# Coder-Yu/SELFRec

Hardware: NVIDIA H100
Metric: XSimGCL yelp2018 train steps/sec (higher is better)
Workload: dtype f32

## Files before the change

selfrec_b200/csrc/common.cuh:

```cuda
#pragma once
#include <cuda_runtime.h>
#include <stdint.h>
#include <stdio.h>
#include <atomic>
#include <functional>
#include <utility>
#include "selfrec_b200.h"

#define SRB_FULL_MASK 0xffffffffu

namespace srb {

void set_error(const char* fmt, ...);
extern std::atomic<long long> g_launches;

inline int check_cuda(cudaError_t e, const char* what) {
  if (e != cudaSuccess) {
    set_error("%s: %s", what, cudaGetErrorString(e));
    return SRB_ERR_CUDA;
  }
  return SRB_OK;
}

inline int post_launch(const char* what) {
  g_launches.fetch_add(1, std::memory_order_relaxed);
  return check_cuda(cudaPeekAtLastError(), what);
}

__device__ __forceinline__ void pdl_wait() { asm volatile("griddepcontrol.wait;" ::: "memory"); }
__device__ __forceinline__ void pdl_trigger() { asm volatile("griddepcontrol.launch_dependents;" ::: "memory"); }

bool pdl_active();

template <typename... KArgs, typename... Args>
inline int launch_kernel(void (*kernel)(KArgs...), dim3 grid, dim3 block, size_t smem, cudaStream_t st, const char* what,
                         Args&&... args) {
  cudaLaunchAttribute attr[1];
  attr[0].id = cudaLaunchAttributeProgrammaticStreamSerialization;
  attr[0].val.programmaticStreamSerializationAllowed = 1;
  cudaLaunchConfig_t cfg = {};
  cfg.gridDim = grid;
  cfg.blockDim = block;
  cfg.dynamicSmemBytes = smem;
  cfg.stream = st;
  cfg.attrs = attr;
  cfg.numAttrs = pdl_active() ? 1 : 0;
  const cudaError_t e = cudaLaunchKernelEx(&cfg, kernel, std::forward<Args>(args)...);
  g_launches.fetch_add(1, std::memory_order_relaxed);
  return check_cuda(e, what);
}

#define SRB_REQUIRE(cond, ...)            \
  do {                                    \
    if (!(cond)) {                        \
      srb::set_error(__VA_ARGS__);        \
      return SRB_ERR_ARG;                 \
    }                                     \
  } while (0)

#define SRB_TRY(expr)                     \
  do {                                    \
    int _rc = (expr);                     \
    if (_rc != SRB_OK) return _rc;        \
  } while (0)

int sm_count();
long long l2_bytes();

struct ScatterSeg {
  const float* src;
  const int32_t* rows;
  const int32_t* n_dev;
  int32_t n;
  int32_t row_off;
  float scale;
  int32_t mod, rem;
  int32_t item_min;
  int32_t item_off;
};
struct ScatterSegs {
  int count;
  ScatterSeg s[16];
};
int scatter_segments(float* dst, int d, const ScatterSegs& segs, cudaStream_t st);

struct SeedRows {
  int32_t user_off[3], item_off[3];
  int32_t user_mod, user_rem;
  int32_t item_min;
};
struct SeedGrads {
  const int32_t* batch;
  int cap, d;
  const float *emb, *l2;
  const float *nce_u[2], *nce_i[2];
  const int32_t *cat, *n_cat;
};
int seed_segments(int model, int n_layers, int layer_cl, const SeedGrads& g, const SeedRows& r, ScatterSegs& segs);
int step_begin(int32_t* step, float* scalars, double lr, double b1, double b2, int32_t* words, int n_words, const int32_t* batch, int cap,
               int d, float* seed, int n_seed, const SeedRows& r, cudaStream_t st);

struct LossRows {
  const int32_t* batch;
  const int32_t *u, *i, *j;
  int32_t item_off;
  const int32_t *uq_u, *uq_i;
  int32_t uq_off[2];
  const int32_t *cat, *n_cat;
  const int32_t* cat_id;
};
struct LossBufs {
  float *g_emb, *g_l2;
  float* g_nce;
  size_t nce_plane;
  float *bpr_scratch, *bpr_losses, *nce_losses;
  void* nce_ws;
  int64_t nce_ws_bytes;
  float* losses;
};
struct ForkRes;
int step_losses(int model, float reg, float l2_div, float tau, float cl_rate, int d, int cap, const float* out, const float* e0,
                const float* v1, const float* v2, const LossRows& r, const LossBufs& o, ForkRes* fork,
                const std::function<int()>& before_nce, SeedGrads& g, cudaStream_t st);

__device__ __forceinline__ void adam_prepare(int32_t* step, float* scalars, double lr, double b1, double b2) {
  const int t = *step + 1;
  *step = t;
  const double bc1 = 1.0 - pow(b1, (double)t);
  const double bc2 = 1.0 - pow(b2, (double)t);
  scalars[0] = (float)(lr / bc1);
  scalars[1] = (float)sqrt(bc2);
}

__device__ __forceinline__ float warp_sum(float v) {
#pragma unroll
  for (int o = 16; o > 0; o >>= 1) v += __shfl_xor_sync(SRB_FULL_MASK, v, o);
  return v;
}

__device__ __forceinline__ float4 ldg4(const float* p) {
  return __ldg(reinterpret_cast<const float4*>(p));
}

__device__ __forceinline__ void st4(float* p, const float4& v) {
  *reinterpret_cast<float4*>(p) = v;
}

__device__ __forceinline__ float4 f4_zero() { return make_float4(0.f, 0.f, 0.f, 0.f); }

__device__ __forceinline__ float4 f4_fma(float a, const float4& x, const float4& acc) {
  return make_float4(fmaf(a, x.x, acc.x), fmaf(a, x.y, acc.y), fmaf(a, x.z, acc.z),
                     fmaf(a, x.w, acc.w));
}

__device__ __forceinline__ float4 f4_add(const float4& a, const float4& b) {
  return make_float4(a.x + b.x, a.y + b.y, a.z + b.z, a.w + b.w);
}

__device__ __forceinline__ float4 f4_scale(float s, const float4& a) {
  return make_float4(s * a.x, s * a.y, s * a.z, s * a.w);
}

__device__ __forceinline__ float f4_dot(const float4& a, const float4& b) {
  return fmaf(a.w, b.w, fmaf(a.z, b.z, fmaf(a.y, b.y, a.x * b.x)));
}

__device__ __forceinline__ float sgnf(float x) {
  return (x > 0.f) ? 1.f : ((x < 0.f) ? -1.f : 0.f);
}

__device__ __forceinline__ uint4 philox4x32_10(uint4 ctr, uint2 key) {
  const uint32_t M0 = 0xD2511F53u, M1 = 0xCD9E8D57u, W0 = 0x9E3779B9u, W1 = 0xBB67AE85u;
#pragma unroll
  for (int r = 0; r < 10; ++r) {
    uint32_t hi0 = __umulhi(M0, ctr.x), lo0 = M0 * ctr.x;
    uint32_t hi1 = __umulhi(M1, ctr.z), lo1 = M1 * ctr.z;
    ctr = make_uint4(hi1 ^ ctr.y ^ key.x, lo1, hi0 ^ ctr.w ^ key.y, lo0);
    key.x += W0;
    key.y += W1;
  }
  return ctr;
}

__device__ __forceinline__ float u32_to_unit(uint32_t x) {
  return (float)(x >> 8) * (1.0f / 16777216.0f);
}

}
```

selfrec_b200/csrc/engine.cu:

```cuda
#include <stdlib.h>
#include <algorithm>
#include <mutex>
#include "spmm_args.cuh"

namespace srb {

static bool pdl_enabled() {
  static const bool on = [] {
    const char* e = getenv("SRB_PDL");
    return !(e && e[0] == '0');
  }();
  return on;
}

static thread_local bool t_pdl = false;
bool pdl_active() { return t_pdl; }

struct PdlScope {
  PdlScope() { t_pdl = pdl_enabled(); }
  ~PdlScope() { t_pdl = false; }
};

struct Ws {
  float* final_;
  float* cl;
  float* v2;
  float* work0;
  float* work1;
  float* acc0;
  float* acc1;
  float* gd;
  float* rsum;
  float* seed;
  int32_t n_seed;
  float* g_emb;
  float* g_l2;
  float* g_nce;
  float* bpr_scratch;
  float* bpr_losses;
  float* nce_losses;
  int32_t* idx_cat;
  int32_t* n_cat;
  int32_t* batch_rows;
  int32_t* n_hub;
  uint32_t* row_mask;
  int32_t* hub_first;
  int32_t* hub_work;
  float* hub_part;
  int32_t hub_cap;
  void* nce_ws;
  int64_t nce_ws_bytes;
};

static int64_t al(int64_t x) { return (x + 255) / 256 * 256; }

static int64_t carve(const srb_step_desc* s, Ws* w, char* base) {
  const int64_t N = (int64_t)s->n_users + s->n_items, d = s->d, B = s->batch_cap;
  const int64_t nd = al(N * d * 4);
  int64_t off = 0;
  auto take = [&](int64_t bytes) {
    char* p = base ? base + off : nullptr;
    off += al(bytes);
    return p;
  };
  const bool graph = s->model != SRB_MODEL_MF;
  const bool two_views = s->model == SRB_MODEL_SIMGCL || s->model == SRB_MODEL_SGL;
  const bool has_cl = s->model == SRB_MODEL_XSIMGCL || two_views;
  const int n_seed = s->model == SRB_MODEL_SGL ? 3 : (s->model == SRB_MODEL_SIMGCL ? 1 : (graph ? 2 : 0));
  float* f_gemb = (float*)take(3 * B * d * 4);
  float* f_gl2 = (float*)take(3 * B * d * 4);
  float* f_gnce = (float*)take(has_cl ? 4 * 2 * B * d * 4 : 0);
  float* f_bs = (float*)take(8 * 4);
  float* f_bl = (float*)take(2 * 4);
  float* f_nl = (float*)take(4 * 4);
  int32_t* i_cat = (int32_t*)take(2 * B * 4);
  int32_t* i_ncat = (int32_t*)take(4);
  int32_t* i_brows = (int32_t*)take(4 * 3 * B * 4);
  int32_t* i_nhub = (int32_t*)take(graph ? 32 + ((N + 31) / 32) * 4 : 32);
  uint32_t* u_mask = (uint32_t*)(i_nhub + 8);
  const int64_t hub_cap = graph ? s->adj.hub.n_work : 0;
  int32_t* i_hfirst = (int32_t*)take(hub_cap ? 3 * B * 4 : 0);
  int32_t* i_hwork = (int32_t*)take(hub_cap * 2 * 4);
  float* f_hpart = (float*)take(hub_cap * d * 4);
  const int64_t nws = has_cl ? srb_infonce_workspace_bytes((int32_t)(2 * B), (int32_t)d, 2) : 0;
  void* v_nws = take(nws);
  float* f_final = (float*)take(graph ? nd : 0);
  float* f_cl = (float*)take(has_cl ? nd : 0);
  float* f_v2 = (float*)take(two_views ? nd : 0);
  float* f_w0 = (float*)take(graph ? nd : 0);
  float* f_w1 = (float*)take(graph ? nd : 0);
  float* f_a0 = (float*)take(nd);
  float* f_a1 = (float*)take(graph ? nd : 0);
  float* f_gd = (float*)take(two_views ? nd : 0);
  float* f_rsum = (float*)take(graph ? nd : 0);
  float* f_seed = (float*)take(n_seed * nd);
  if (w) {
    w->final_ = f_final;
    w->cl = f_cl;
    w->v2 = f_v2;
    w->work0 = f_w0;
    w->work1 = f_w1;
    w->acc0 = f_a0;
    w->acc1 = f_a1;
    w->gd = f_gd;
    w->rsum = f_rsum;
    w->seed = f_seed;
    w->n_seed = n_seed;
    w->g_emb = f_gemb;
    w->g_l2 = f_gl2;
    w->g_nce = f_gnce;
    w->bpr_scratch = f_bs;
    w->bpr_losses = f_bl;
    w->nce_losses = f_nl;
    w->idx_cat = i_cat;
    w->n_cat = i_ncat;
    w->batch_rows = i_brows;
    w->n_hub = i_nhub;
    w->row_mask = u_mask;
    w->hub_first = i_hfirst;
    w->hub_work = i_hwork;
    w->hub_part = f_hpart;
    w->hub_cap = (int32_t)hub_cap;
    w->nce_ws = v_nws;
    w->nce_ws_bytes = nws;
  }
  return off;
}

__global__ void build_cat_idx_kernel(const int32_t* batch, int cap, int n_users, int32_t* idx_cat, int32_t* n_cat) {
  pdl_wait();
  pdl_trigger();
  const int nu = min(batch[1], cap), ni = min(batch[2], cap);
  const int32_t* uu = batch + SRB_BATCH_HEADER + 3 * cap;
  const int32_t* ui = uu + cap;
  for (int t = blockIdx.x * blockDim.x + threadIdx.x; t < nu + ni; t += gridDim.x * blockDim.x)
    idx_cat[t] = (t < nu) ? uu[t] : n_users + ui[t - nu];
  if (blockIdx.x == 0 && threadIdx.x == 0) *n_cat = nu + ni;
}

__global__ void __launch_bounds__(256) build_batch_rows_kernel(const int32_t* batch, int cap, int n_users, const int32_t* rowptr,
                                                               int32_t* rows, int32_t* counters, uint32_t* row_mask,
                                                               int32_t* hub_first, int32_t* hub_work, int hub_cap) {
  const int t = blockIdx.x * blockDim.x + threadIdx.x;
  pdl_wait();
  pdl_trigger();
  const int b = min(batch[0], cap);
  const int sec = t / cap, k = t % cap;
  if (sec >= 3 || k >= b) return;
  const int32_t* u = batch + SRB_BATCH_HEADER;
  const int row = (sec == 0) ? u[k] : n_users + u[sec * cap + k];
  const uint32_t bit = 1u << (row & 31);
  if (atomicOr(row_mask + (row >> 5), bit) & bit) return;
  list_batch_row(row, rowptr[row + 1] - rowptr[row], 0, rows, 3 * cap, counters, hub_first, hub_work, hub_cap);
}

template <bool OWNED>
__global__ void __launch_bounds__(256) step_begin_kernel(int32_t* step, float* scalars, double lr, double b1, double b2, int32_t* words,
                                                         int n_words, const int32_t* batch, int cap, int d, float* seed, int n_seed,
                                                         const SeedRows r) {
  pdl_wait();
  pdl_trigger();
  const int t = blockIdx.x * blockDim.x + threadIdx.x;
  if (t == 0) adam_prepare(step, scalars, lr, b1, b2);
  if (t < n_words) words[t] = 0;
  const int k0 = t / (d / 4), c = (t % (d / 4)) * 4;
  const int sec = k0 / cap, k = k0 % cap;
  if (sec >= 3 || k >= min(batch[0], cap)) return;
  const int id = batch[SRB_BATCH_HEADER + sec * cap + k];
  const bool owned = OWNED && sec == 0;
  if (owned && id % r.user_mod != r.user_rem) return;
  for (int q = 0; q < n_seed; ++q) {
    const int row = id + (sec == 0 ? r.user_off[q] : r.item_off[q]);
    st4(seed + (size_t)(owned ? row / r.user_mod : row) * d + c, f4_zero());
  }
}

int step_begin(int32_t* step, float* scalars, double lr, double b1, double b2, int32_t* words, int n_words, const int32_t* batch, int cap,
               int d, float* seed, int n_seed, const SeedRows& r, cudaStream_t st) {
  const int threads = std::max(n_words, 3 * cap * (d / 4));
  return launch_kernel(r.user_mod > 0 ? step_begin_kernel<true> : step_begin_kernel<false>, (threads + 255) / 256, 256, 0, st,
                       "step_begin_kernel", step, scalars, lr, b1, b2, words, n_words, batch, cap, d, seed, n_seed, r);
}

__global__ void finalize_losses_kernel(const float* bpr_losses, const float* nce_losses, int n_nce, float cl_rate, float* out) {
  pdl_wait();
  pdl_trigger();
  float cl = 0.f;
  for (int q = 0; q < n_nce; ++q) cl += nce_losses[q];
  cl *= cl_rate;
  out[0] = bpr_losses[0];
  out[1] = bpr_losses[1];
  out[2] = cl;
  out[3] = bpr_losses[0] + bpr_losses[1] + cl;
}

int seed_segments(int model, int n_layers, int layer_cl, const SeedGrads& g, const SeedRows& r, ScatterSegs& segs) {
  const int B = g.cap, L = n_layers;
  const size_t plane = (size_t)B * g.d;
  const int32_t* rows = g.batch + SRB_BATCH_HEADER;
  const int32_t* n_dev = g.batch;
  const float cm = 1.f / (float)((model == SRB_MODEL_LIGHTGCN || model == SRB_MODEL_SGL) ? L + 1 : L);
  segs.count = 0;
  auto add = [&](int t, bool item, const float* src, const int32_t* idx, const int32_t* n, int cap, float scale) {
    segs.s[segs.count++] = {src, idx, n, cap, item ? r.item_off[t] : r.user_off[t], scale, item ? 0 : r.user_mod, item ? 0 : r.user_rem};
  };
  auto add_bpr = [&](int t, const float* src, float scale) {
    add(t, false, src, rows, n_dev, B, scale);
    add(t, true, src + plane, rows + B, n_dev, B, scale);
    add(t, true, src + 2 * plane, rows + 2 * B, n_dev, B, scale);
  };
  auto add_nce = [&](int t, int view, float scale) {
    add(t, false, g.nce_u[view], rows + 3 * B, n_dev + 1, B, scale);
    add(t, true, g.nce_i[view], rows + 4 * B, n_dev + 2, B, scale);
  };
  int g_level = -1;
  switch (model) {
    case SRB_MODEL_LIGHTGCN:
      add_bpr(0, g.emb, cm);
      add_bpr(1, g.emb, cm);
      add_bpr(1, g.l2, 1.f);
      g_level = 0;
      break;
    case SRB_MODEL_XSIMGCL:
      g_level = (layer_cl >= 1 && layer_cl <= L) ? layer_cl : 0;
      for (int t = 0; t < (g_level ? 2 : 1); ++t) {
        add_bpr(t, g.emb, cm);
        add_nce(t, 0, cm);
      }
      add_nce(1, 1, 1.f);
      break;
    case SRB_MODEL_SIMGCL:
      add_bpr(0, g.emb, cm);
      add_nce(0, 0, cm);
      add_nce(0, 1, cm);
      break;
    case SRB_MODEL_SGL:
      for (int t = 0; t < 2; ++t) {
        add(t, false, g.nce_u[t], g.cat, g.n_cat, 2 * B, cm);
        segs.s[segs.count - 1].item_min = r.item_min;
        segs.s[segs.count - 1].item_off = r.item_min > 0 ? r.item_off[t] : 0;
      }
      add_bpr(2, g.emb, cm);
      break;
  }
  return g_level;
}

static int spmm_simple(const srb_step_desc* s, const srb_graph_csr* g, const float* x, float* y, const float* extra,
                       bool adam, cudaStream_t st, const uint32_t* col_mask = nullptr, const float* seed = nullptr,
                       const uint32_t* seed_mask = nullptr) {
  SpmmArgs a;
  SRB_TRY(graph_args(*g, s->n_users + s->n_items, s->n_users + s->n_items, s->d, x, a));
  a.col_mask = col_mask;
  a.Y = y;
  a.extra = extra;
  a.seed_mask = seed_mask;
  a.seed = seed;
  if (adam) {
    a.ap = s->params;
    a.am = s->adam_m;
    a.av = s->adam_v;
    a.ascal = s->scalars;
    a.b2 = (float)s->beta2;
    a.w1 = (float)(1.0 - s->beta1);
    a.w2 = (float)(1.0 - s->beta2);
    a.aeps = s->adam_eps;
  }
  return launch_spmm(a, s->d, st);
}

struct ForkRes {
  cudaStream_t side;
  cudaEvent_t fork, join;
  bool ok;
};
static ForkRes* fork_res(const srb_step_desc* s, ForkRes* own) {
  if (s->fork_stream && s->fork_event && s->join_event) {
    own->side = (cudaStream_t)s->fork_stream;
    own->fork = (cudaEvent_t)s->fork_event;
    own->join = (cudaEvent_t)s->join_event;
    own->ok = true;
    return own;
  }
  static ForkRes res[64] = {};
  static std::mutex mu;
  int dev = 0;
  if (cudaGetDevice(&dev) != cudaSuccess || dev < 0 || dev >= 64) return nullptr;
  std::lock_guard<std::mutex> lock(mu);
  ForkRes& r = res[dev];
  if (!r.ok) {
    if (cudaStreamCreateWithFlags(&r.side, cudaStreamNonBlocking) != cudaSuccess) return nullptr;
    if (cudaEventCreateWithFlags(&r.fork, cudaEventDisableTiming) != cudaSuccess) return nullptr;
    if (cudaEventCreateWithFlags(&r.join, cudaEventDisableTiming) != cudaSuccess) return nullptr;
    r.ok = true;
  }
  return &r;
}

int step_losses(int model, float reg, float l2_div, float tau, float cl_rate, int d, int cap, const float* out, const float* e0,
                const float* v1, const float* v2, const LossRows& r, const LossBufs& o, ForkRes* fork,
                const std::function<int()>& before_nce, SeedGrads& g, cudaStream_t st) {
  const bool lg = model == SRB_MODEL_LIGHTGCN, xs = model == SRB_MODEL_XSIMGCL, sg = model == SRB_MODEL_SIMGCL;
  if (fork) {
    SRB_TRY(check_cuda(cudaEventRecord(fork->fork, st), "fork record"));
    SRB_TRY(check_cuda(cudaStreamWaitEvent(fork->side, fork->fork, 0), "fork wait"));
  }
  srb_bpr_desc p = {};
  p.emb = out;
  p.l2_emb = lg ? e0 : out;
  p.n_users = r.item_off;
  p.d = d;
  p.u_idx = r.u;
  p.i_idx = r.i;
  p.j_idx = r.j;
  p.b_dev = r.batch;
  p.b = cap;
  p.emb_scale = 1.f;
  p.reg = reg;
  p.l2_terms = (sg || xs) ? 2 : 3;
  p.l2_div = l2_div;
  p.grad_scale = 1.f;
  p.losses = o.bpr_losses;
  p.g_emb = o.g_emb;
  p.g_l2 = lg ? o.g_l2 : nullptr;
  p.scratch = o.bpr_scratch;
  SRB_TRY(srb_bpr_l2_fwd_bwd(&p, fork ? fork->side : st));
  if (fork) SRB_TRY(check_cuda(cudaEventRecord(fork->join, fork->side), "join record"));
  if (before_nce) SRB_TRY(before_nce());

  g = SeedGrads{r.batch, cap, d, o.g_emb, p.g_l2, {}, {}, nullptr, nullptr};
  srb_infonce_desc q = {};
  q.d = d;
  q.b_cos = 1;
  q.temperature = tau;
  q.workspace = o.nce_ws;
  q.workspace_bytes = o.nce_ws_bytes;
  if (xs || sg) {
    const float* t1 = xs ? out : v1;
    const float* t2 = xs ? v1 : v2;
    float* gp[4];
    for (int k = 0; k < 4; ++k) gp[k] = o.g_nce + k * o.nce_plane;
    q.n_problems = 2;
    q.prob[0] = {t1, t2, r.uq_off[0], r.uq_off[0], 1.f, 1.f, r.uq_u, r.batch + 1, cap, cl_rate, gp[0], gp[1], o.nce_losses + 0};
    q.prob[1] = {t1, t2, r.uq_off[1], r.uq_off[1], 1.f, 1.f, r.uq_i, r.batch + 2, cap, cl_rate, gp[2], gp[3], o.nce_losses + 1};
    g.nce_u[0] = gp[0];
    g.nce_u[1] = gp[1];
    g.nce_i[0] = gp[2];
    g.nce_i[1] = gp[3];
  } else if (model == SRB_MODEL_SGL) {
    float* g2 = o.g_nce + (size_t)2 * cap * d;
    q.n_problems = 1;
    q.prob[0] = {v1, v2, 0, 0, 1.f, 1.f, r.cat, r.n_cat, 2 * cap, cl_rate, o.g_nce, g2, o.nce_losses + 0};
    g.nce_u[0] = o.g_nce;
    g.nce_u[1] = g2;
    g.cat = r.cat_id;
    g.n_cat = r.n_cat;
  }
  if (q.n_problems) SRB_TRY(srb_infonce_fwd_bwd(&q, st));
  if (fork) SRB_TRY(check_cuda(cudaStreamWaitEvent(st, fork->join, 0), "join wait"));
  return launch_kernel(finalize_losses_kernel, 1, 1, 0, st, "finalize_losses_kernel", o.bpr_losses, o.nce_losses, q.n_problems, cl_rate,
                       o.losses);
}

static int run_chain(const srb_step_desc* s, const Ws& w, const srb_graph_csr* g, const float* F, const float* G, int g_level,
                     bool include_ego, float* out, const float* extra, cudaStream_t st) {
  const int L = s->n_layers;
  const float* x = g_level == L ? G : F;
  for (int k = L - 1; k >= 1; --k) {
    float* y = (x == w.acc0) ? w.acc1 : w.acc0;
    SRB_TRY(spmm_simple(s, g, x, y, nullptr, false, st, k == L - 1 ? w.row_mask : nullptr, g_level == k ? G : F, w.row_mask));
    x = y;
  }
  const float* seed0 = g_level == 0 ? G : (include_ego ? F : nullptr);
  return spmm_simple(s, g, x, out, extra, out == nullptr, st, L == 1 ? w.row_mask : nullptr, seed0, w.row_mask);
}

static ScatterSeg seg(const float* src, const int32_t* rows, const int32_t* n_dev, int n, int row_off, float scale) {
  ScatterSeg g = {src, rows, n_dev, n, row_off, scale};
  return g;
}

static int encoder(const srb_step_desc* s, const Ws& w, const srb_graph_csr* g, bool include_ego, int noise_mode, int view,
                   int layer_cl, float* final_out, float* cl_out, cudaStream_t st, const float* x1 = nullptr) {
  srb_encoder_desc e = {};
  e.rowptr = g->rowptr;
  e.colidx = g->colidx;
  e.vals = g->vals;
  e.row_order = g->row_order;
  e.n_long_rows = g->n_long_rows;
  e.n_vlong_rows = g->n_vlong_rows;
  e.hub = g->hub;
  e.n = s->n_users + s->n_items;
  e.d = s->d;
  e.n_layers = s->n_layers;
  e.include_ego = include_ego;
  e.layer_cl = layer_cl;
  e.noise_mode = noise_mode;
  if (noise_mode == 1) e.noise = s->noise + (size_t)view * s->n_layers * e.n * e.d;
  e.eps = s->eps;
  e.philox_seed = s->philox_seed;
  e.philox_offset = noise_offset(view, 0);
  e.philox_step_dev = s->step_dev;
  e.E0 = s->params;
  if (cl_out && layer_cl == s->n_layers) {
    e.final_out = final_out;
  } else {
    e.last_rows = w.batch_rows;
    e.n_last_rows = 3 * s->batch_cap;
    e.last_rows_nv_dev = w.n_hub;
    e.last_rows_hub = srb_hub_split{0, w.hub_cap, w.hub_first, w.hub_work, w.hub_part};
    e.last_rows_out = final_out;
    e.final_out = w.rsum;
  }
  e.cl_out = cl_out;
  e.work0 = w.work0;
  e.work1 = w.work1;
  e.x1 = x1;
  return srb_encoder_forward(&e, st);
}

static int perturb_rows(const srb_step_desc* s, const float* x, float* out, int view, cudaStream_t st) {
  const int N = s->n_users + s->n_items;
  SpmmArgs a;
  SRB_TRY(graph_args(s->adj, N, N, s->d, x, a));
  a.Y = out;
  a.noise_mode = s->noise_mode;
  if (s->noise_mode == 1) a.noise = s->noise + (size_t)view * s->n_layers * N * s->d;
  a.eps = s->eps;
  const uint64_t poff = noise_offset(view, 0);
  a.pkey = make_uint2((uint32_t)s->philox_seed, (uint32_t)(s->philox_seed >> 32));
  a.poff = make_uint2((uint32_t)poff, (uint32_t)(poff >> 32));
  a.pstep = s->step_dev;
  return launch_rows_epilogue(a, s->d, st);
}

}

extern "C" int64_t srb_step_workspace_bytes(int32_t model, int32_t n, int32_t d, int32_t batch_cap, int32_t n_hub_work) {
  srb_step_desc s = {};
  s.adj.hub.n_work = n_hub_work > 0 ? n_hub_work : 0;
  s.model = model;
  s.n_users = n;
  s.n_items = 0;
  s.d = d;
  s.batch_cap = batch_cap;
  return srb::carve(&s, nullptr, nullptr);
}

extern "C" int srb_train_step(const srb_step_desc* s, void* stream) {
  using namespace srb;
  SRB_REQUIRE(s != nullptr, "step: null desc");
  SRB_REQUIRE(s->model >= SRB_MODEL_MF && s->model <= SRB_MODEL_SGL, "step: unknown model %d", s->model);
  SRB_REQUIRE(s->d == 32 || s->d == 64 || s->d == 128, "step: unsupported d=%d (32, 64, 128)", s->d);
  SRB_REQUIRE(s->n_users > 0 && s->n_items > 0 && s->batch_cap > 0, "step: bad sizes");
  SRB_REQUIRE(s->params && s->adam_m && s->adam_v && s->step_dev && s->scalars && s->losses && s->batch, "step: null pointer");
  SRB_REQUIRE(s->model == SRB_MODEL_MF || s->n_layers >= 1, "step: graph models need n_layers >= 1");
  SRB_REQUIRE(s->model == SRB_MODEL_MF || (s->adj.rowptr && s->adj.colidx && s->adj.vals), "step: null adjacency");
  const int N = s->n_users + s->n_items;
  const int64_t need = srb_step_workspace_bytes(s->model, N, s->d, s->batch_cap, s->model != SRB_MODEL_MF ? s->adj.hub.n_work : 0);
  SRB_REQUIRE(s->workspace && s->workspace_bytes >= need, "step: workspace too small (%lld < %lld)",
              (long long)s->workspace_bytes, (long long)need);
  SRB_REQUIRE(((uintptr_t)s->workspace & 255) == 0, "step: workspace must be 256-byte aligned");
  Ws w;
  carve(s, &w, (char*)s->workspace);
  cudaStream_t st = (cudaStream_t)stream;
  const int B = s->batch_cap, d = s->d, U = s->n_users, L = s->n_layers;
  const int32_t* u_idx = s->batch + SRB_BATCH_HEADER;
  const int32_t* i_idx = u_idx + B;
  const int32_t* j_idx = i_idx + B;
  const int32_t* uq_u = j_idx + B;
  const int32_t* uq_i = uq_u + B;
  const int32_t* b_dev = s->batch;
  const SeedRows rows = {{0, N, 2 * N}, {U, N + U, 2 * N + U}, 0, 0};

  PdlScope pdl;

  if (s->model != SRB_MODEL_MF) {
    const int n_words = 8 + (U + s->n_items + 31) / 32;
    SRB_TRY(step_begin(s->step_dev, s->scalars, s->lr, s->beta1, s->beta2, w.n_hub, n_words, s->batch, B, d, w.seed, w.n_seed, rows, st));
    SRB_TRY(launch_kernel(build_batch_rows_kernel, (3 * B + 255) / 256, 256, 0, st, "build_batch_rows_kernel", s->batch, B, U, s->adj.rowptr,
                          w.batch_rows, w.n_hub, w.row_mask, w.hub_cap ? w.hub_first : nullptr, w.hub_work, w.hub_cap));
  } else {
    SRB_TRY(srb_adam_prepare(s->step_dev, s->scalars, s->lr, s->beta1, s->beta2, stream));
  }
  const float* table = s->params;
  switch (s->model) {
    case SRB_MODEL_MF: break;
    case SRB_MODEL_LIGHTGCN:
      SRB_TRY(encoder(s, w, &s->adj, true, 0, 0, 0, w.final_, nullptr, st));
      table = w.final_;
      break;
    case SRB_MODEL_XSIMGCL:
      SRB_REQUIRE(s->noise_mode == 1 || s->noise_mode == 2, "step: XSimGCL needs noise_mode 1 or 2");
      SRB_REQUIRE(s->noise_mode != 1 || s->noise, "step: noise tensor missing");
      SRB_TRY(encoder(s, w, &s->adj, false, s->noise_mode, 0, s->layer_cl, w.final_, w.cl, st));
      table = w.final_;
      break;
    case SRB_MODEL_SIMGCL:
      SRB_REQUIRE(s->noise_mode == 1 || s->noise_mode == 2, "step: SimGCL needs noise_mode 1 or 2");
      SRB_REQUIRE(s->noise_mode != 1 || s->noise, "step: noise tensor missing");
      if (L >= 2) {
        SRB_TRY(spmm_simple(s, &s->adj, s->params, w.acc0, nullptr, false, st));
        SRB_TRY(perturb_rows(s, w.acc0, w.acc1, 0, st));
        SRB_TRY(perturb_rows(s, w.acc0, w.gd, 1, st));
        SRB_TRY(encoder(s, w, &s->adj, false, 0, 0, 0, w.final_, nullptr, st, w.acc0));
        SRB_TRY(encoder(s, w, &s->adj, false, s->noise_mode, 0, 0, w.cl, nullptr, st, w.acc1));
        SRB_TRY(encoder(s, w, &s->adj, false, s->noise_mode, 1, 0, w.v2, nullptr, st, w.gd));
      } else {
        SRB_TRY(encoder(s, w, &s->adj, false, 0, 0, 0, w.final_, nullptr, st));
        SRB_TRY(encoder(s, w, &s->adj, false, s->noise_mode, 0, 0, w.cl, nullptr, st));
        SRB_TRY(encoder(s, w, &s->adj, false, s->noise_mode, 1, 0, w.v2, nullptr, st));
      }
      table = w.final_;
      break;
    case SRB_MODEL_SGL:
      SRB_REQUIRE(s->adj_view[0].rowptr && s->adj_view[1].rowptr, "step: SGL needs two view graphs");
      SRB_TRY(encoder(s, w, &s->adj, true, 0, 0, 0, w.final_, nullptr, st));
      SRB_TRY(encoder(s, w, &s->adj_view[0], true, 0, 0, 0, w.cl, nullptr, st));
      SRB_TRY(encoder(s, w, &s->adj_view[1], true, 0, 0, 0, w.v2, nullptr, st));
      table = w.final_;
      break;
  }

  ForkRes fk_own = {};
  ForkRes* fk = (s->model == SRB_MODEL_XSIMGCL || s->model == SRB_MODEL_SIMGCL || s->model == SRB_MODEL_SGL) ? fork_res(s, &fk_own) : nullptr;
  std::function<int()> build_cat;
  if (s->model == SRB_MODEL_SGL)
    build_cat = [&] { return launch_kernel(build_cat_idx_kernel, 8, 256, 0, st, "build_cat_idx_kernel", s->batch, B, U, w.idx_cat, w.n_cat); };
  const LossRows lr = {s->batch, u_idx, i_idx, j_idx, U, uq_u, uq_i, {0, U}, w.idx_cat, w.n_cat, w.idx_cat};
  const LossBufs lb = {w.g_emb, w.g_l2, w.g_nce, (size_t)2 * B * d, w.bpr_scratch, w.bpr_losses, w.nce_losses, w.nce_ws, w.nce_ws_bytes, s->losses};
  SeedGrads gr;
  SRB_TRY(step_losses(s->model, s->reg, s->l2_div, s->tau, s->cl_rate, d, B, table, s->params, w.cl, w.v2, lr, lb, fk, build_cat, gr, st));

  const size_t plane = (size_t)B * d;
  if (s->model == SRB_MODEL_MF) {
    const size_t bytes = (size_t)N * d * 4;
    SRB_TRY(check_cuda(cudaMemsetAsync(w.acc0, 0, bytes, st), "mf memset"));
    ScatterSegs sg;
    sg.count = 3;
    sg.s[0] = seg(w.g_emb, u_idx, b_dev, B, 0, 1.f);
    sg.s[1] = seg(w.g_emb + plane, i_idx, b_dev, B, U, 1.f);
    sg.s[2] = seg(w.g_emb + 2 * plane, j_idx, b_dev, B, U, 1.f);
    SRB_TRY(scatter_segments(w.acc0, d, sg, st));
    return srb_adam_step(s->params, s->adam_m, s->adam_v, w.acc0, (int64_t)N * d, s->scalars, s->beta1, s->beta2, s->adam_eps,
                         stream);
  }
  auto seed_table = [&](int t) { return w.seed + (size_t)t * N * d; };
  ScatterSegs sg = {};
  const int g_level = seed_segments(s->model, L, s->layer_cl, gr, rows, sg);
  SRB_TRY(scatter_segments(w.seed, d, sg, st));
  if (s->model != SRB_MODEL_SGL)
    return run_chain(s, w, &s->adj, seed_table(0), g_level >= 0 ? seed_table(1) : nullptr, g_level, s->model == SRB_MODEL_LIGHTGCN,
                     nullptr, nullptr, st);
  SRB_TRY(run_chain(s, w, &s->adj_view[0], seed_table(0), nullptr, -1, true, w.gd, nullptr, st));
  SRB_TRY(run_chain(s, w, &s->adj_view[1], seed_table(1), nullptr, -1, true, w.gd, w.gd, st));
  return run_chain(s, w, &s->adj, seed_table(2), nullptr, -1, true, nullptr, w.gd, st);
}
```

selfrec_b200/csrc/infonce.cu:

```cuda
#include "common.cuh"
#include "infonce_tc.cuh"

namespace srb {

constexpr int NCE_T = 64;
constexpr int NCE_MAX_SPLITS = 8;

struct NceProblem {
  const float* table1;
  const float* table2;
  int32_t row_off1, row_off2;
  float scale1, scale2;
  const int32_t* idx;
  const int32_t* n_dev;
  int32_t n;
  float weight;
  float* g1;
  float* g2;
  float* loss;
  float* V1;
  float* V2;
  float* V1T;
  float* V2T;
  float* inv1;
  float* inv2;
  float* diag;
  float* part_m;
  float* part_l;
  float* dV1;
  float* dV2;
  float* loss_acc;
  float* lse;
};

struct NceArgs {
  int32_t n_problems;
  int32_t np;
  int32_t splits;
  int32_t b_cos;
  float inv_tau;
  NceProblem p[4];
};

__device__ __forceinline__ float tf32_rna(float x) {
  uint32_t r;
  asm("cvt.rna.tf32.f32 %0, %1;" : "=r"(r) : "f"(x));
  return __uint_as_float(r);
}

__device__ __forceinline__ int nce_n(const NceProblem& p) { return p.n_dev ? min(*p.n_dev, p.n) : p.n; }

template <int D>
__global__ void __launch_bounds__(256) nce_prep_kernel(const NceArgs a) {
  pdl_wait();
  pdl_trigger();
  const NceProblem& p = a.p[blockIdx.y];
  const int lane = threadIdx.x & 31;
  const int i = blockIdx.x * (blockDim.x >> 5) + (threadIdx.x >> 5);
  if (i >= a.np) return;
  const int n = nce_n(p);
  if (blockIdx.x == 0 && threadIdx.x == 0) *p.loss_acc = 0.f;
  constexpr int Q = (D + 127) / 128;
  float4 v1[Q], v2[Q];
  float s1 = 0.f, s2 = 0.f, s12 = 0.f;
  if (i < n) {
    const int r = p.idx[i];
#pragma unroll
    for (int q = 0; q < Q; ++q) {
      const int c = lane * 4 + q * 128;
      v1[q] = (c < D) ? f4_scale(p.scale1, ldg4(p.table1 + (size_t)(r + p.row_off1) * D + c)) : f4_zero();
      v2[q] = (c < D) ? f4_scale(p.scale2, ldg4(p.table2 + (size_t)(r + p.row_off2) * D + c)) : f4_zero();
      s1 += f4_dot(v1[q], v1[q]);
      s2 += f4_dot(v2[q], v2[q]);
    }
  } else {
#pragma unroll
    for (int q = 0; q < Q; ++q) v1[q] = f4_zero(), v2[q] = f4_zero();
  }
  s1 = warp_sum(s1);
  s2 = warp_sum(s2);
  float i1 = 1.f, i2 = 1.f;
  if (a.b_cos) {
    i1 = 1.f / fmaxf(sqrtf(s1), 1e-12f);
    i2 = 1.f / fmaxf(sqrtf(s2), 1e-12f);
  }
#pragma unroll
  for (int q = 0; q < Q; ++q) {
    const int c = lane * 4 + q * 128;
    if (a.b_cos) {
      const float n1 = fmaxf(sqrtf(s1), 1e-12f), n2 = fmaxf(sqrtf(s2), 1e-12f);
      v1[q] = make_float4(v1[q].x / n1, v1[q].y / n1, v1[q].z / n1, v1[q].w / n1);
      v2[q] = make_float4(v2[q].x / n2, v2[q].y / n2, v2[q].z / n2, v2[q].w / n2);
    }
    s12 += f4_dot(v1[q], v2[q]);
    if (c < D) {
      st4(p.V1 + (size_t)i * D + c, v1[q]);
      st4(p.V2 + (size_t)i * D + c, v2[q]);
      st4(p.dV1 + (size_t)i * D + c, f4_zero());
      st4(p.dV2 + (size_t)i * D + c, f4_zero());
      p.V1T[(size_t)(c + 0) * a.np + i] = v1[q].x;
      p.V1T[(size_t)(c + 1) * a.np + i] = v1[q].y;
      p.V1T[(size_t)(c + 2) * a.np + i] = v1[q].z;
      p.V1T[(size_t)(c + 3) * a.np + i] = v1[q].w;
      p.V2T[(size_t)(c + 0) * a.np + i] = v2[q].x;
      p.V2T[(size_t)(c + 1) * a.np + i] = v2[q].y;
      p.V2T[(size_t)(c + 2) * a.np + i] = v2[q].z;
      p.V2T[(size_t)(c + 3) * a.np + i] = v2[q].w;
    }
  }
  s12 = warp_sum(s12);
  if (lane == 0) {
    p.inv1[i] = i1;
    p.inv2[i] = i2;
    p.diag[i] = s12 * a.inv_tau;
  }
}

__global__ void __launch_bounds__(256) nce_prep_tc_kernel(const NceArgs a) {
  pdl_wait();
  pdl_trigger();
  constexpr int D = 64;
  __shared__ float t1[32][D + 1], t2[32][D + 1];
  const NceProblem& p = a.p[blockIdx.y];
  const int lane = threadIdx.x & 31, warp = threadIdx.x >> 5;
  const int i0 = blockIdx.x * 32;
  const int n = nce_n(p);
  if (blockIdx.x == 0 && threadIdx.x == 0) *p.loss_acc = 0.f;
  const size_t nd = (size_t)a.np * D;
  float* hi = p.dV2 + nd;
  float* lo = hi + 4 * nd;
#pragma unroll 1
  for (int rr = 0; rr < 4; ++rr) {
    const int il = warp * 4 + rr, i = i0 + il;
    const int c = lane * 2;
    float2 v1 = make_float2(0.f, 0.f), v2 = make_float2(0.f, 0.f);
    if (i < n) {
      const int r = p.idx[i];
      v1 = *reinterpret_cast<const float2*>(p.table1 + (size_t)(r + p.row_off1) * D + c);
      v2 = *reinterpret_cast<const float2*>(p.table2 + (size_t)(r + p.row_off2) * D + c);
      v1.x *= p.scale1, v1.y *= p.scale1, v2.x *= p.scale2, v2.y *= p.scale2;
    }
    const float s1 = warp_sum(v1.x * v1.x + v1.y * v1.y);
    const float s2 = warp_sum(v2.x * v2.x + v2.y * v2.y);
    float i1 = 1.f, i2 = 1.f;
    if (a.b_cos) {
      const float n1 = fmaxf(sqrtf(s1), 1e-12f), n2 = fmaxf(sqrtf(s2), 1e-12f);
      i1 = 1.f / n1, i2 = 1.f / n2;
      v1.x /= n1, v1.y /= n1, v2.x /= n2, v2.y /= n2;
    }
    const float s12 = warp_sum(v1.x * v2.x + v1.y * v2.y);
    const size_t o = (size_t)i * D + c;
    *reinterpret_cast<float2*>(p.V1 + o) = v1;
    *reinterpret_cast<float2*>(p.V2 + o) = v2;
    *reinterpret_cast<float2*>(p.dV1 + o) = make_float2(0.f, 0.f);
    *reinterpret_cast<float2*>(p.dV2 + o) = make_float2(0.f, 0.f);
    const float2 h1 = make_float2(tf32_rna(v1.x), tf32_rna(v1.y)), h2 = make_float2(tf32_rna(v2.x), tf32_rna(v2.y));
    *reinterpret_cast<float2*>(hi + o) = h1;
    *reinterpret_cast<float2*>(hi + nd + o) = h2;
    *reinterpret_cast<float2*>(lo + o) = make_float2(v1.x - h1.x, v1.y - h1.y);
    *reinterpret_cast<float2*>(lo + nd + o) = make_float2(v2.x - h2.x, v2.y - h2.y);
    t1[il][c] = v1.x, t1[il][c + 1] = v1.y;
    t2[il][c] = v2.x, t2[il][c + 1] = v2.y;
    if (lane == 0) {
      p.inv1[i] = i1;
      p.inv2[i] = i2;
      const float dg = s12 * a.inv_tau;
      p.diag[i] = dg;
      p.part_l[i] = expf(dg - a.inv_tau);
    }
  }
  __syncthreads();
  for (int e = threadIdx.x; e < D * 32; e += 256) {
    const int dc = e >> 5, il = e & 31;
    const size_t o = (size_t)dc * a.np + i0 + nce_tperm(il);
    const float x1 = t1[il][dc], x2 = t2[il][dc];
    const float g1 = tf32_rna(x1), g2 = tf32_rna(x2);
    hi[2 * nd + o] = g1;
    hi[3 * nd + o] = g2;
    lo[2 * nd + o] = x1 - g1;
    lo[3 * nd + o] = x2 - g2;
  }
}

template <int D>
__device__ __forceinline__ void load_kmajor(float (*dst)[NCE_T], const float* T, int np, int col0) {
  for (int e = threadIdx.x; e < D * (NCE_T / 4); e += blockDim.x) {
    const int k = e / (NCE_T / 4), c4 = e % (NCE_T / 4);
    *reinterpret_cast<float4*>(&dst[k][c4 * 4]) = *reinterpret_cast<const float4*>(T + (size_t)k * np + col0 + c4 * 4);
  }
}

template <int D>
__device__ __forceinline__ void load_rowmajor(float (*dst)[D], const float* V, int row0) {
  for (int e = threadIdx.x; e < NCE_T * (D / 4); e += blockDim.x) {
    const int r = e / (D / 4), c4 = e % (D / 4);
    *reinterpret_cast<float4*>(&dst[r][c4 * 4]) = *reinterpret_cast<const float4*>(V + (size_t)(row0 + r) * D + c4 * 4);
  }
}

template <int D>
__device__ __forceinline__ void s_tile(const float (*AsT)[NCE_T], const float (*BsT)[NCE_T], int ty, int tx, float (&s)[4][4]) {
#pragma unroll
  for (int r = 0; r < 4; ++r)
#pragma unroll
    for (int c = 0; c < 4; ++c) s[r][c] = 0.f;
#pragma unroll 8
  for (int k = 0; k < D; ++k) {
    const float4 av = *reinterpret_cast<const float4*>(&AsT[k][ty * 4]);
    const float4 bv = *reinterpret_cast<const float4*>(&BsT[k][tx * 4]);
    const float ar[4] = {av.x, av.y, av.z, av.w};
    const float bc[4] = {bv.x, bv.y, bv.z, bv.w};
#pragma unroll
    for (int r = 0; r < 4; ++r)
#pragma unroll
      for (int c = 0; c < 4; ++c) s[r][c] = fmaf(ar[r], bc[c], s[r][c]);
  }
}

template <int D>
struct NceLseSmem {
  float AsT[D][NCE_T];
  float BsT[D][NCE_T];
};

template <int D>
__global__ void __launch_bounds__(256) nce_lse_kernel(const NceArgs a) {
  pdl_wait();
  pdl_trigger();
  extern __shared__ __align__(16) unsigned char smem_raw[];
  NceLseSmem<D>& sm = *reinterpret_cast<NceLseSmem<D>*>(smem_raw);
  const NceProblem& p = a.p[blockIdx.z];
  const int n = nce_n(p);
  const int i0 = blockIdx.x * NCE_T;
  if (i0 >= n) return;
  const int split = blockIdx.y;
  const int ty = threadIdx.x >> 4, tx = threadIdx.x & 15;
  load_kmajor<D>(sm.AsT, p.V1T, a.np, i0);
  float m[4], l[4];
#pragma unroll
  for (int r = 0; r < 4; ++r) m[r] = -INFINITY, l[r] = 0.f;
  const int ntiles = (n + NCE_T - 1) / NCE_T;
  const float L2E = 1.4426950408889634f;
  for (int jt = split; jt < ntiles; jt += a.splits) {
    const int j0 = jt * NCE_T;
    __syncthreads();
    load_kmajor<D>(sm.BsT, p.V2T, a.np, j0);
    __syncthreads();
    float s[4][4];
    s_tile<D>(sm.AsT, sm.BsT, ty, tx, s);
#pragma unroll
    for (int r = 0; r < 4; ++r) {
      float tm = -INFINITY;
#pragma unroll
      for (int c = 0; c < 4; ++c) {
        s[r][c] = (j0 + tx * 4 + c < n) ? s[r][c] * a.inv_tau : -INFINITY;
        tm = fmaxf(tm, s[r][c]);
      }
      const float mn = fmaxf(m[r], tm);
      if (mn > -INFINITY) {
        float acc = 0.f;
#pragma unroll
        for (int c = 0; c < 4; ++c) acc += exp2f((s[r][c] - mn) * L2E);
        l[r] = l[r] * exp2f((m[r] - mn) * L2E) + acc;
        m[r] = mn;
      }
    }
  }
#pragma unroll
  for (int r = 0; r < 4; ++r) {
#pragma unroll
    for (int o = 8; o > 0; o >>= 1) {
      const float mo = __shfl_xor_sync(SRB_FULL_MASK, m[r], o);
      const float lo = __shfl_xor_sync(SRB_FULL_MASK, l[r], o);
      const float mn = fmaxf(m[r], mo);
      if (mn > -INFINITY) {
        l[r] = l[r] * exp2f((m[r] - mn) * L2E) + lo * exp2f((mo - mn) * L2E);
        m[r] = mn;
      }
    }
    if (tx == 0) {
      const int i = i0 + ty * 4 + r;
      p.part_m[(size_t)split * a.np + i] = m[r];
      p.part_l[(size_t)split * a.np + i] = l[r];
    }
  }
}

template <int D>
struct NceGradSmem {
  float AsT[D][NCE_T];
  float BsT[D][NCE_T];
  float Ar[NCE_T][D];
  float Br[NCE_T][D];
  float Gs[NCE_T][NCE_T];
  float GsT[NCE_T][NCE_T];
  float lse[NCE_T];
  float red[8];
};

template <int D>
__global__ void __launch_bounds__(256) nce_grad_kernel(const NceArgs a) {
  pdl_wait();
  pdl_trigger();
  constexpr int CW = D / 16;
  extern __shared__ __align__(16) unsigned char smem_raw[];
  NceGradSmem<D>& sm = *reinterpret_cast<NceGradSmem<D>*>(smem_raw);
  const NceProblem& p = a.p[blockIdx.z];
  const int n = nce_n(p);
  const int i0 = blockIdx.x * NCE_T;
  if (i0 >= n) return;
  const int split = blockIdx.y;
  const int ty = threadIdx.x >> 4, tx = threadIdx.x & 15;
  const float L2E = 1.4426950408889634f;
  load_kmajor<D>(sm.AsT, p.V1T, a.np, i0);
  load_rowmajor<D>(sm.Ar, p.V1, i0);
  if (threadIdx.x < NCE_T) {
    const int i = i0 + threadIdx.x;
    float M = -INFINITY;
    for (int s = 0; s < a.splits; ++s) M = fmaxf(M, p.part_m[(size_t)s * a.np + i]);
    float Lsum = 0.f;
    for (int s = 0; s < a.splits; ++s) {
      const float ms = p.part_m[(size_t)s * a.np + i];
      if (ms > -INFINITY) Lsum += p.part_l[(size_t)s * a.np + i] * exp2f((ms - M) * L2E);
    }
    const float lse = (i < n) ? M + logf(Lsum) : 0.f;
    sm.lse[threadIdx.x] = lse;
    float contrib = (split == 0 && i < n) ? lse - p.diag[i] : 0.f;
    contrib = warp_sum(contrib);
    if ((threadIdx.x & 31) == 0) sm.red[threadIdx.x >> 5] = contrib;
  }
  __syncthreads();
  if (threadIdx.x == 0 && split == 0) atomicAdd(p.loss_acc, sm.red[0] + sm.red[1]);
  const float gscale = p.weight * a.inv_tau / (float)n;
  float o1[4][CW];
#pragma unroll
  for (int r = 0; r < 4; ++r)
#pragma unroll
    for (int q = 0; q < CW; ++q) o1[r][q] = 0.f;
  const int ntiles = (n + NCE_T - 1) / NCE_T;
  for (int jt = split; jt < ntiles; jt += a.splits) {
    const int j0 = jt * NCE_T;
    __syncthreads();
    load_kmajor<D>(sm.BsT, p.V2T, a.np, j0);
    load_rowmajor<D>(sm.Br, p.V2, j0);
    __syncthreads();
    float s[4][4];
    s_tile<D>(sm.AsT, sm.BsT, ty, tx, s);
#pragma unroll
    for (int r = 0; r < 4; ++r) {
      const int i = i0 + ty * 4 + r;
      const float lse = sm.lse[ty * 4 + r];
#pragma unroll
      for (int c = 0; c < 4; ++c) {
        const int j = j0 + tx * 4 + c;
        float g = 0.f;
        if (i < n && j < n) {
          g = exp2f((s[r][c] * a.inv_tau - lse) * L2E);
          if (i == j) g -= 1.f;
          g *= gscale;
        }
        s[r][c] = g;
      }
      *reinterpret_cast<float4*>(&sm.Gs[ty * 4 + r][tx * 4]) = make_float4(s[r][0], s[r][1], s[r][2], s[r][3]);
    }
#pragma unroll
    for (int c = 0; c < 4; ++c) {
      const int jl = tx * 4 + c;
      *reinterpret_cast<float4*>(&sm.GsT[jl][((ty ^ (jl >> 2)) & 15) * 4]) = make_float4(s[0][c], s[1][c], s[2][c], s[3][c]);
    }
    __syncthreads();
#pragma unroll 4
    for (int j = 0; j < NCE_T; ++j) {
      const float4 av = *reinterpret_cast<const float4*>(&sm.GsT[j][((ty ^ (j >> 2)) & 15) * 4]);
      const float ar[4] = {av.x, av.y, av.z, av.w};
      float bq[CW];
#pragma unroll
      for (int q = 0; q < CW; ++q) bq[q] = sm.Br[j][tx * CW + q];
#pragma unroll
      for (int r = 0; r < 4; ++r)
#pragma unroll
        for (int q = 0; q < CW; ++q) o1[r][q] = fmaf(ar[r], bq[q], o1[r][q]);
    }
    float qv[4][CW];
#pragma unroll
    for (int r = 0; r < 4; ++r)
#pragma unroll
      for (int q = 0; q < CW; ++q) qv[r][q] = 0.f;
#pragma unroll 4
    for (int i = 0; i < NCE_T; ++i) {
      const float4 av = *reinterpret_cast<const float4*>(&sm.Gs[i][ty * 4]);
      const float ar[4] = {av.x, av.y, av.z, av.w};
      float bq[CW];
#pragma unroll
      for (int q = 0; q < CW; ++q) bq[q] = sm.Ar[i][tx * CW + q];
#pragma unroll
      for (int r = 0; r < 4; ++r)
#pragma unroll
        for (int q = 0; q < CW; ++q) qv[r][q] = fmaf(ar[r], bq[q], qv[r][q]);
    }
#pragma unroll
    for (int r = 0; r < 4; ++r) {
      const int j = j0 + ty * 4 + r;
      if (j < n) {
#pragma unroll
        for (int q = 0; q < CW; ++q) atomicAdd(p.dV2 + (size_t)j * D + tx * CW + q, qv[r][q]);
      }
    }
  }
#pragma unroll
  for (int r = 0; r < 4; ++r) {
    const int i = i0 + ty * 4 + r;
    if (i < n) {
#pragma unroll
      for (int q = 0; q < CW; ++q) atomicAdd(p.dV1 + (size_t)i * D + tx * CW + q, o1[r][q]);
    }
  }
}

template <int D>
__global__ void __launch_bounds__(256) nce_finish_kernel(const NceArgs a) {
  pdl_wait();
  pdl_trigger();
  const NceProblem& p = a.p[blockIdx.y];
  const int lane = threadIdx.x & 31;
  const int i = blockIdx.x * (blockDim.x >> 5) + (threadIdx.x >> 5);
  const int n = nce_n(p);
  if (blockIdx.x == 0 && threadIdx.x == 0) *p.loss = (n > 0) ? *p.loss_acc / (float)n : 0.f;
  if (i >= n) return;
  constexpr int Q = (D + 127) / 128;
#pragma unroll 1
  for (int side = 0; side < 2; ++side) {
    const float* V = side ? p.V2 : p.V1;
    const float* dV = side ? p.dV2 : p.dV1;
    float* g = side ? p.g2 : p.g1;
    const float inv = side ? p.inv2[i] : p.inv1[i];
    float4 vh[Q], dv[Q];
    float dot = 0.f;
#pragma unroll
    for (int q = 0; q < Q; ++q) {
      const int c = lane * 4 + q * 128;
      vh[q] = (c < D) ? *reinterpret_cast<const float4*>(V + (size_t)i * D + c) : f4_zero();
      dv[q] = (c < D) ? *reinterpret_cast<const float4*>(dV + (size_t)i * D + c) : f4_zero();
      dot += f4_dot(vh[q], dv[q]);
    }
    dot = warp_sum(dot);
#pragma unroll
    for (int q = 0; q < Q; ++q) {
      const int c = lane * 4 + q * 128;
      if (c >= D) continue;
      float4 o = dv[q];
      if (a.b_cos) {
        o = make_float4((dv[q].x - vh[q].x * dot) * inv, (dv[q].y - vh[q].y * dot) * inv, (dv[q].z - vh[q].z * dot) * inv,
                        (dv[q].w - vh[q].w * dot) * inv);
      }
      st4(g + (size_t)i * D + c, o);
    }
  }
}

static inline int64_t align_up(int64_t x, int64_t a) { return (x + a - 1) / a * a; }
static inline int nce_np(int n) { return (int)align_up(n > 0 ? n : 1, 128); }

static int64_t nce_problem_floats(int np, int d) {
  return 14ll * np * d + 4ll * np + 2ll * NCE_MAX_SPLITS * np + 64;
}

__global__ void __launch_bounds__(256) nce_tc_finish_kernel(const NceArgs a) {
  pdl_wait();
  pdl_trigger();
  constexpr int D = 64;
  const NceProblem& p = a.p[blockIdx.y];
  const int lane = threadIdx.x & 31;
  const int i = blockIdx.x * (blockDim.x >> 5) + (threadIdx.x >> 5);
  const int n = nce_n(p);
  if (blockIdx.x == 0 && threadIdx.x == 0) *p.loss = (n > 0) ? *p.loss_acc / (float)n : 0.f;
  if (i >= n) return;
  const float li = p.part_l[i];
  const float pii = expf(p.diag[i] - a.inv_tau) / li;
  const float gs = p.weight * a.inv_tau / (float)n;
  const float cd = (pii - 1.f) * gs;
  const float2 v1 = *reinterpret_cast<const float2*>(p.V1 + (size_t)i * D + lane * 2);
  const float2 v2 = *reinterpret_cast<const float2*>(p.V2 + (size_t)i * D + lane * 2);
#pragma unroll 1
  for (int side = 0; side < 2; ++side) {
    const float2 vh = side ? v2 : v1;
    const float2 vo = side ? v1 : v2;
    float2 dv = *reinterpret_cast<const float2*>((side ? p.dV2 : p.dV1) + (size_t)i * D + lane * 2);
    if (side == 0) dv.x *= gs / li, dv.y *= gs / li;
    dv.x = fmaf(cd, vo.x, dv.x);
    dv.y = fmaf(cd, vo.y, dv.y);
    const float dot = warp_sum(vh.x * dv.x + vh.y * dv.y);
    const float inv = side ? p.inv2[i] : p.inv1[i];
    float2 o = dv;
    if (a.b_cos) o = make_float2((dv.x - vh.x * dot) * inv, (dv.y - vh.y * dot) * inv);
    *reinterpret_cast<float2*>((side ? p.g2 : p.g1) + (size_t)i * D + lane * 2) = o;
  }
}

static int nce_launch_tc(const NceArgs& a, int n_problems, cudaStream_t st) {
  const int np = a.np;
  const int d = NT_D;
  {
    dim3 grid(np / 32, n_problems);
    SRB_TRY(launch_kernel(nce_prep_tc_kernel, grid, 256, 0, st, "nce_prep_tc_kernel", a));
  }
  NtMaps maps;
  NtArgs t;
  t.np = np;
  t.inv_tau = a.inv_tau;
  const int row_blocks = np / NT_T;
  int splits = sm_count() / (row_blocks * n_problems);
  if (splits < 1) splits = 1;
  if (splits > NT_MAX_SPLITS) splits = NT_MAX_SPLITS;
  if (splits > row_blocks) splits = row_blocks;
  t.splits = splits;
  const long long nd = (long long)np * d;
  for (int q = 0; q < n_problems; ++q) {
    const NceProblem& p = a.p[q];
    float* hi = p.dV2 + nd;
    float* lo = hi + 4 * nd;
    for (int h = 0; h < 2; ++h) {
      float* r = h ? lo : hi;
      SRB_REQUIRE(make_tmap_f32_rows(&maps.v1r[q][h], r, (uint64_t)np, d, NT_T) == 0 &&
                      make_tmap_f32_rows(&maps.v2r[q][h], r + nd, (uint64_t)np, d, NT_T) == 0 &&
                      make_tmap_f32_rows(&maps.v1c[q][h], r, (uint64_t)np, d, NT_C) == 0 &&
                      make_tmap_f32_rows(&maps.v2c[q][h], r + nd, (uint64_t)np, d, NT_C) == 0 &&
                      make_tmap_f32_rows(&maps.v1t[q][h], r + 2 * nd, (uint64_t)d, (uint64_t)np, NT_D) == 0 &&
                      make_tmap_f32_rows(&maps.v2t[q][h], r + 3 * nd, (uint64_t)d, (uint64_t)np, NT_D) == 0,
                  "infonce: cuTensorMapEncodeTiled failed");
    }
    NtProblem& o = t.p[q];
    o.n = p.n;
    o.n_dev = p.n_dev;
    o.weight = p.weight;
    o.diag = p.diag;
    o.lsum = p.part_l;
    o.dV1 = p.dV1;
    o.dV2 = p.dV2;
    o.loss_acc = p.loss_acc;
  }
  for (int q = n_problems; q < 2; ++q) {
    for (int h = 0; h < 2; ++h) {
      maps.v1r[q][h] = maps.v1r[0][h];
      maps.v2r[q][h] = maps.v2r[0][h];
      maps.v1c[q][h] = maps.v1c[0][h];
      maps.v2c[q][h] = maps.v2c[0][h];
      maps.v1t[q][h] = maps.v1t[0][h];
      maps.v2t[q][h] = maps.v2t[0][h];
    }
    t.p[q] = t.p[0];
  }
  const size_t smem = NtSmem::total + 1024;
  static bool attr_done = false;
  if (!attr_done) {
    SRB_TRY(check_cuda(cudaFuncSetAttribute(nce_tc_kernel<1>, cudaFuncAttributeMaxDynamicSharedMemorySize, (int)smem), "nce tc attr"));
    SRB_TRY(check_cuda(cudaFuncSetAttribute(nce_tc_kernel<2>, cudaFuncAttributeMaxDynamicSharedMemorySize, (int)smem), "nce tc attr"));
    attr_done = true;
  }
  dim3 grid(row_blocks, splits, n_problems);
  SRB_TRY(launch_kernel(nce_tc_kernel<1>, grid, NT_THREADS, smem, st, "nce_tc_kernel<pass_a>", maps, t));
  SRB_TRY(launch_kernel(nce_tc_kernel<2>, grid, NT_THREADS, smem, st, "nce_tc_kernel<pass_b>", maps, t));
  return launch_kernel(nce_tc_finish_kernel, dim3((np + 7) / 8, n_problems), 256, 0, st, "nce_tc_finish_kernel", a);
}

template <int D>
static int nce_launch(const NceArgs& a, int n_problems, cudaStream_t st) {
  const int np = a.np;
  {
    dim3 grid((np + 7) / 8, n_problems);
    SRB_TRY(launch_kernel(nce_prep_kernel<D>, grid, 256, 0, st, "nce_prep_kernel", a));
  }
  {
    static bool attr_done = false;
    if (!attr_done) {
      SRB_TRY(check_cuda(cudaFuncSetAttribute(nce_lse_kernel<D>, cudaFuncAttributeMaxDynamicSharedMemorySize, (int)sizeof(NceLseSmem<D>)), "nce lse smem attr"));
      SRB_TRY(check_cuda(cudaFuncSetAttribute(nce_grad_kernel<D>, cudaFuncAttributeMaxDynamicSharedMemorySize, (int)sizeof(NceGradSmem<D>)), "nce grad smem attr"));
      attr_done = true;
    }
    dim3 grid(np / NCE_T, a.splits, n_problems);
    SRB_TRY(launch_kernel(nce_lse_kernel<D>, grid, 256, sizeof(NceLseSmem<D>), st, "nce_lse_kernel", a));
    SRB_TRY(launch_kernel(nce_grad_kernel<D>, grid, 256, sizeof(NceGradSmem<D>), st, "nce_grad_kernel", a));
  }
  {
    dim3 grid((np + 7) / 8, n_problems);
    SRB_TRY(launch_kernel(nce_finish_kernel<D>, grid, 256, 0, st, "nce_finish_kernel", a));
  }
  return SRB_OK;
}

}

extern "C" int64_t srb_infonce_workspace_bytes(int32_t max_n, int32_t d, int32_t n_problems) {
  if (max_n < 0 || d <= 0 || n_problems <= 0) return 0;
  return srb::nce_problem_floats(srb::nce_np(max_n), d) * 4 * n_problems;
}

extern "C" int srb_infonce_fwd_bwd(const srb_infonce_desc* d, void* stream) {
  SRB_REQUIRE(d != nullptr, "infonce: null desc");
  SRB_REQUIRE(d->n_problems >= 1 && d->n_problems <= 4, "infonce: n_problems must be 1..4");
  SRB_REQUIRE(d->temperature > 0.f, "infonce: temperature must be positive");
  SRB_REQUIRE(d->d == 32 || d->d == 64 || d->d == 128, "infonce: unsupported d=%d (32, 64, 128)", d->d);
  int max_n = 0;
  for (int q = 0; q < d->n_problems; ++q) {
    const srb_infonce_problem& s = d->prob[q];
    SRB_REQUIRE(s.table1 && s.table2 && s.idx && s.g1 && s.g2 && s.loss, "infonce: null pointer in problem %d", q);
    SRB_REQUIRE(s.n >= 0, "infonce: negative n");
    if (s.n > max_n) max_n = s.n;
  }
  SRB_REQUIRE(d->workspace && d->workspace_bytes >= srb_infonce_workspace_bytes(max_n, d->d, d->n_problems),
              "infonce: workspace too small (%lld < %lld)", (long long)d->workspace_bytes,
              (long long)srb_infonce_workspace_bytes(max_n, d->d, d->n_problems));
  if (max_n == 0) {
    for (int q = 0; q < d->n_problems; ++q)
      SRB_TRY(srb::check_cuda(cudaMemsetAsync(d->prob[q].loss, 0, 4, (cudaStream_t)stream), "infonce memset"));
    return SRB_OK;
  }
  srb::NceArgs a;
  a.n_problems = d->n_problems;
  a.np = srb::nce_np(max_n);
  a.b_cos = d->b_cos;
  a.inv_tau = 1.0f / d->temperature;
  const int row_blocks = a.np / srb::NCE_T;
  int splits = (2 * srb::sm_count() + row_blocks * d->n_problems - 1) / (row_blocks * d->n_problems);
  if (splits < 1) splits = 1;
  if (splits > srb::NCE_MAX_SPLITS) splits = srb::NCE_MAX_SPLITS;
  if (splits > row_blocks) splits = row_blocks;
  a.splits = splits;
  float* w = reinterpret_cast<float*>(d->workspace);
  const int64_t per = srb::nce_problem_floats(a.np, d->d);
  for (int q = 0; q < d->n_problems; ++q) {
    const srb_infonce_problem& s = d->prob[q];
    srb::NceProblem& p = a.p[q];
    p.table1 = s.table1;
    p.table2 = s.table2;
    p.row_off1 = s.row_off1;
    p.row_off2 = s.row_off2;
    p.scale1 = s.scale1;
    p.scale2 = s.scale2;
    p.idx = s.idx;
    p.n_dev = s.n_dev;
    p.n = s.n;
    p.weight = s.weight;
    p.g1 = s.g1;
    p.g2 = s.g2;
    p.loss = s.loss;
    float* base = w + per * q;
    const int64_t nd = (int64_t)a.np * d->d;
    p.V1 = base;
    p.V2 = base + nd;
    p.V1T = base + 2 * nd;
    p.V2T = base + 3 * nd;
    p.dV1 = base + 4 * nd;
    p.dV2 = base + 5 * nd;
    float* t = base + 14 * nd;
    p.inv1 = t;
    p.inv2 = t + a.np;
    p.diag = t + 2 * a.np;
    p.part_m = t + 3 * a.np;
    p.part_l = t + 3 * a.np + (int64_t)srb::NCE_MAX_SPLITS * a.np;
    p.lse = t + 3 * a.np + 2ll * srb::NCE_MAX_SPLITS * a.np;
    p.loss_acc = p.lse + a.np;
  }
  cudaStream_t st = (cudaStream_t)stream;
  if (d->d == 64 && d->b_cos && d->n_problems <= 2 && a.inv_tau <= 40.f) return srb::nce_launch_tc(a, d->n_problems, st);
  switch (d->d) {
    case 32: return srb::nce_launch<32>(a, d->n_problems, st);
    case 64: return srb::nce_launch<64>(a, d->n_problems, st);
    default: return srb::nce_launch<128>(a, d->n_problems, st);
  }
}
```

selfrec_b200/csrc/spmm.cu:

```cuda
#include "spmm_args.cuh"

namespace srb {

__device__ __forceinline__ void st4_cs(float* p, const float4& v, int stream) {
  if (stream) __stcs(reinterpret_cast<float4*>(p), v);
  else st4(p, v);
}

__device__ __forceinline__ void st4_peer(float* p, const float4& v, int mc) {
  if (mc) asm volatile("multimem.st.weak.global.v4.f32 [%0], {%1, %2, %3, %4};" ::"l"(p), "f"(v.x), "f"(v.y), "f"(v.z), "f"(v.w) : "memory");
  else st4(p, v);
}

__device__ __forceinline__ float4 ldg4_if(const float* p, bool pred) {
  float4 r = f4_zero();
  asm("{\n\t.reg .pred q;\n\tsetp.ne.b32 q, %5, 0;\n\t@q ld.global.nc.v4.f32 {%0, %1, %2, %3}, [%4];\n\t}"
      : "+f"(r.x), "+f"(r.y), "+f"(r.z), "+f"(r.w)
      : "l"(p), "r"((int)pred));
  return r;
}

template <int D>
__device__ __forceinline__ void spmm_epilogue(const SpmmArgs& a, int row, int gl, float4 acc0, float4 acc1, bool valid) {
  constexpr int LPR = D / 8;
  constexpr int HALF = D / 2;
  {
    if (a.stage_peer[0]) {
      if (!valid) return;
      int o = 0;
#pragma unroll 1
      while (row >= a.stage_bounds[o + 1]) ++o;
      float* dst = a.stage_peer[o] + ((size_t)a.stage_rank * a.stage_cap + (row - a.stage_bounds[o])) * D + gl * 4;
      st4(dst, acc0);
      st4(dst + HALF, acc1);
      return;
    }
    const size_t off = (size_t)row * D + gl * 4;
    float4 y0 = acc0, y1 = acc1;
    if (a.extra && valid) {
      y0 = f4_fma(a.extra_scale, *reinterpret_cast<const float4*>(a.extra + off), y0);
      y1 = f4_fma(a.extra_scale, *reinterpret_cast<const float4*>(a.extra + off + HALF), y1);
    }
    if (a.seed && valid) {
      if ((__ldg(a.seed_mask + (row >> 5)) >> (row & 31)) & 1u) {
        y0 = f4_add(y0, *reinterpret_cast<const float4*>(a.seed + off));
        y1 = f4_add(y1, *reinterpret_cast<const float4*>(a.seed + off + HALF));
      }
    }
    if (a.noise_mode) {
      float4 n0 = f4_zero(), n1 = f4_zero();
      if (a.noise_mode == 1) {
        if (valid) {
          n0 = ldg4(a.noise + off);
          n1 = ldg4(a.noise + off + HALF);
        }
      } else {
        const uint32_t stp = a.pstep ? (uint32_t)*a.pstep : 0u;
        const uint32_t grow = (uint32_t)(a.noise_row_base + row * a.noise_row_stride);
        const uint32_t vw = a.poff.y << 16;
        const uint4 r0 = philox4x32_10(make_uint4(grow, (uint32_t)gl | vw, a.poff.x, stp), a.pkey);
        const uint4 r1 = philox4x32_10(make_uint4(grow, (uint32_t)(gl + LPR) | vw, a.poff.x, stp), a.pkey);
        n0 = make_float4(u32_to_unit(r0.x), u32_to_unit(r0.y), u32_to_unit(r0.z), u32_to_unit(r0.w));
        n1 = make_float4(u32_to_unit(r1.x), u32_to_unit(r1.y), u32_to_unit(r1.z), u32_to_unit(r1.w));
      }
      float ss = f4_dot(n0, n0) + f4_dot(n1, n1);
#pragma unroll
      for (int o = LPR / 2; o > 0; o >>= 1) ss += __shfl_xor_sync(SRB_FULL_MASK, ss, o);
      const float nrm = fmaxf(sqrtf(ss), 1e-12f);
#define SRB_PERT(Y, N, F) Y.F += sgnf(Y.F) * (N.F / nrm) * a.eps;
      SRB_PERT(y0, n0, x) SRB_PERT(y0, n0, y) SRB_PERT(y0, n0, z) SRB_PERT(y0, n0, w)
      SRB_PERT(y1, n1, x) SRB_PERT(y1, n1, y) SRB_PERT(y1, n1, z) SRB_PERT(y1, n1, w)
#undef SRB_PERT
    }
    if (!valid) return;
    if (a.Y) {
      st4_cs(a.Y + off, y0, a.stream);
      st4_cs(a.Y + off + HALF, y1, a.stream);
    }
    if (a.world > 0 && a.peer[0]) {
#pragma unroll 1
      for (int g = 0; g < a.world; ++g) {
        st4_peer(a.peer[g] + off, y0, a.peer_mc);
        st4_peer(a.peer[g] + off + HALF, y1, a.peer_mc);
      }
    }
    if (a.sum_out) {
      float4 s0 = y0, s1 = y1;
      if (a.sum_in) {
        float4 t0 = *reinterpret_cast<const float4*>(a.sum_in + off);
        float4 t1 = *reinterpret_cast<const float4*>(a.sum_in + off + HALF);
#pragma unroll
        for (int j = 0; j < 3; ++j) {
          if (!a.sum_add[j]) break;
          t0 = f4_add(*reinterpret_cast<const float4*>(a.sum_add[j] + off), t0);
          t1 = f4_add(*reinterpret_cast<const float4*>(a.sum_add[j] + off + HALF), t1);
        }
        s0 = f4_add(s0, t0);
        s1 = f4_add(s1, t1);
      }
      s0 = f4_scale(a.sum_scale, s0);
      s1 = f4_scale(a.sum_scale, s1);
      st4_cs(a.sum_out + off, s0, a.stream);
      st4_cs(a.sum_out + off + HALF, s1, a.stream);
      if (a.world > 0 && a.peer_sum[0]) {
#pragma unroll 1
        for (int g = 0; g < a.world; ++g) {
          st4_peer(a.peer_sum[g] + off, s0, a.peer_mc);
          st4_peer(a.peer_sum[g] + off + HALF, s1, a.peer_mc);
        }
      }
    }
    if (a.ap) {
      const float step_size = a.ascal[0];
      const float bc2_sqrt = a.ascal[1];
#pragma unroll
      for (int h = 0; h < 2; ++h) {
        const size_t o2 = off + h * HALF;
        const float4 g = h ? y1 : y0;
        float4 p4 = *reinterpret_cast<const float4*>(a.ap + o2);
        float4 m = *reinterpret_cast<const float4*>(a.am + o2);
        float4 v4 = *reinterpret_cast<const float4*>(a.av + o2);
#define SRB_ADAM1(F)                                          \
  m.F = m.F + a.w1 * (g.F - m.F);                             \
  v4.F = v4.F * a.b2;                                         \
  v4.F = v4.F + (a.w2 * g.F) * g.F;                           \
  p4.F = p4.F - step_size * (m.F / (sqrtf(v4.F) / bc2_sqrt + a.aeps));
        SRB_ADAM1(x) SRB_ADAM1(y) SRB_ADAM1(z) SRB_ADAM1(w)
#undef SRB_ADAM1
        st4(a.ap + o2, p4);
        st4_cs(a.am + o2, m, a.stream);
        st4_cs(a.av + o2, v4, a.stream);
        if (a.world > 0 && a.peer_p[0]) {
#pragma unroll 1
          for (int g = 0; g < a.world; ++g) st4_peer(a.peer_p[g] + o2, p4, a.peer_mc);
        }
      }
    }
  }
}

template <int D, bool MASKED>
__device__ __forceinline__ void spmm_gather(const SpmmArgs& a, int p, int end, int stride, int gl, float4& acc0, float4& acc1) {
  constexpr int LPR = D / 8;
  constexpr int HALF = D / 2;
  constexpr int SB = LPR < 4 ? LPR : 4;
  constexpr bool masked = MASKED;
  const int lane = threadIdx.x & 31;
  const int gbase = lane - gl;
  int c = 0;
  float v = 0.f;
  bool hit = false;
  if (p + gl < end) {
    c = a.stream ? __ldcs(a.colidx + p + gl) : __ldg(a.colidx + p + gl);
    v = a.stream ? __ldcs(a.vals + p + gl) : __ldg(a.vals + p + gl);
    if (masked) hit = (__ldg(a.col_mask + (c >> 5)) >> (c & 31)) & 1u;
  }
  while (__any_sync(SRB_FULL_MASK, p < end)) {
    int cn = 0;
    float vn = 0.f;
    bool hitn = false;
    if (p + stride + gl < end) {
      cn = a.stream ? __ldcs(a.colidx + p + stride + gl) : __ldg(a.colidx + p + stride + gl);
      vn = a.stream ? __ldcs(a.vals + p + stride + gl) : __ldg(a.vals + p + stride + gl);
      if (masked) hitn = (__ldg(a.col_mask + (cn >> 5)) >> (cn & 31)) & 1u;
    }
    if (!masked) {
#pragma unroll
      for (int j0 = 0; j0 < LPR; j0 += SB) {
        if (j0 > 0 && !__any_sync(SRB_FULL_MASK, p + j0 < end)) break;
        float vv[SB];
        float4 x0[SB], x1[SB];
#pragma unroll
        for (int j = 0; j < SB; ++j) {
          const int cc = __shfl_sync(SRB_FULL_MASK, c, j0 + j, LPR);
          vv[j] = __shfl_sync(SRB_FULL_MASK, v, j0 + j, LPR);
          const float* xr = a.X + (size_t)cc * D + gl * 4;
          x0[j] = ldg4(xr);
          x1[j] = ldg4(xr + HALF);
        }
#pragma unroll
        for (int j = 0; j < SB; ++j) {
          acc0 = f4_fma(vv[j], x0[j], acc0);
          acc1 = f4_fma(vv[j], x1[j], acc1);
        }
      }
    } else {
      uint32_t gm = (__ballot_sync(SRB_FULL_MASK, hit) >> gbase) & ((1u << LPR) - 1u);
      while (__any_sync(SRB_FULL_MASK, gm != 0)) {
        float vv[SB];
        float4 x0[SB], x1[SB];
#pragma unroll
        for (int j = 0; j < SB; ++j) {
          const int src = gm ? (__ffs(gm) - 1) : 0;
          const bool live = gm != 0;
          gm &= gm - 1;
          const int cc = __shfl_sync(SRB_FULL_MASK, c, gbase + src);
          const float vs = __shfl_sync(SRB_FULL_MASK, v, gbase + src);
          vv[j] = live ? vs : 0.f;
          const float* xr = a.X + (size_t)cc * D + gl * 4;
          x0[j] = ldg4_if(xr, live);
          x1[j] = ldg4_if(xr + HALF, live);
        }
#pragma unroll
        for (int j = 0; j < SB; ++j) {
          acc0 = f4_fma(vv[j], x0[j], acc0);
          acc1 = f4_fma(vv[j], x1[j], acc1);
        }
      }
    }
    c = cn;
    v = vn;
    hit = hitn;
    p += stride;
  }
}

__device__ __forceinline__ void xor_reduce_groups(float4& acc0, float4& acc1, int lpr) {
  for (int o = lpr; o < 32; o <<= 1) {
    acc0.x += __shfl_xor_sync(SRB_FULL_MASK, acc0.x, o);
    acc0.y += __shfl_xor_sync(SRB_FULL_MASK, acc0.y, o);
    acc0.z += __shfl_xor_sync(SRB_FULL_MASK, acc0.z, o);
    acc0.w += __shfl_xor_sync(SRB_FULL_MASK, acc0.w, o);
    acc1.x += __shfl_xor_sync(SRB_FULL_MASK, acc1.x, o);
    acc1.y += __shfl_xor_sync(SRB_FULL_MASK, acc1.y, o);
    acc1.z += __shfl_xor_sync(SRB_FULL_MASK, acc1.z, o);
    acc1.w += __shfl_xor_sync(SRB_FULL_MASK, acc1.w, o);
  }
}

template <int D, bool MASKED>
__global__ void __launch_bounds__(256) spmm_hub_kernel(const SpmmArgs a) {
  constexpr int LPR = D / 8;
  const int lane = threadIdx.x & 31;
  const int wib = threadIdx.x >> 5;
  const int grp = lane / LPR;
  const int gl = lane % LPR;
  pdl_wait();
  pdl_trigger();
  const int n_work = a.seg ? a.n_cta : (a.n_vlong_dev ? min(a.n_vlong_dev[4], a.n_work) : a.n_work);
  __shared__ float4 part[8][2][LPR];
  for (int k = blockIdx.x; k < n_work; k += gridDim.x) {
    int w = k, beg, end;
    if (a.seg) {
      w = __ldg(a.order_cta + k);
      beg = __ldg(a.seg + 2 * w);
      end = __ldg(a.seg + 2 * w + 1);
    } else {
      const int row = __ldg(a.hub_work + 2 * w);
      const int ci = __ldg(a.hub_work + 2 * w + 1);
      const int rbeg = __ldg(a.rowptr + row), rend = __ldg(a.rowptr + row + 1);
      beg = min(rend, rbeg + ci * SRB_HUB_CHUNK);
      end = min(rend, beg + SRB_HUB_CHUNK);
    }
    const int per = ((end - beg + 255) / 256) * 32;
    const int wbeg = beg + wib * per;
    const int wend = min(end, wbeg + per);
    float4 acc0 = f4_zero(), acc1 = f4_zero();
    spmm_gather<D, MASKED>(a, wbeg + grp * LPR, wend, 32, gl, acc0, acc1);
    xor_reduce_groups(acc0, acc1, LPR);
    if (grp == 0) {
      part[wib][0][gl] = acc0;
      part[wib][1][gl] = acc1;
    }
    __syncthreads();
    if (wib == 0 && grp == 0) {
      acc0 = f4_zero();
      acc1 = f4_zero();
#pragma unroll
      for (int q = 0; q < 8; ++q) {
        acc0 = f4_add(acc0, part[q][0][gl]);
        acc1 = f4_add(acc1, part[q][1][gl]);
      }
      float* dst = a.hub_part + (size_t)w * D + gl * 4;
      st4(dst, acc0);
      st4(dst + D / 2, acc1);
    }
    __syncthreads();
  }
}

template <int D, bool MASKED>
__global__ void __launch_bounds__(256) spmm_seg_warp_kernel(const SpmmArgs a) {
  constexpr int LPR = D / 8;
  const int lane = threadIdx.x & 31;
  const int grp = lane / LPR;
  const int gl = lane % LPR;
  const int warp0 = (blockIdx.x * blockDim.x + threadIdx.x) >> 5;
  const int nwarps = (gridDim.x * blockDim.x) >> 5;
  pdl_wait();
  pdl_trigger();
  for (int k = warp0; k < a.n_warp; k += nwarps) {
    const int w = __ldg(a.order_warp + k);
    const int beg = __ldg(a.seg + 2 * w), end = __ldg(a.seg + 2 * w + 1);
    float4 acc0 = f4_zero(), acc1 = f4_zero();
    spmm_gather<D, MASKED>(a, beg + grp * LPR, end, 32, gl, acc0, acc1);
    xor_reduce_groups(acc0, acc1, LPR);
    if (grp == 0) {
      float* dst = a.hub_part + (size_t)w * D + gl * 4;
      st4(dst, acc0);
      st4(dst + D / 2, acc1);
    }
  }
}

template <int D>
__global__ void __launch_bounds__(256) spmm_hub_finish_kernel(const SpmmArgs a) {
  constexpr int LPR = D / 8;
  constexpr int RPW = 32 / LPR;
  const int lane = threadIdx.x & 31;
  const int grp = lane / LPR;
  const int gl = lane % LPR;
  const int warp0 = (blockIdx.x * blockDim.x + threadIdx.x) >> 5;
  const int nwarps = (gridDim.x * blockDim.x) >> 5;
  pdl_wait();
  pdl_trigger();
  const int n_huge = a.n_vlong_dev ? min(a.n_vlong_dev[0], a.n_rows) : a.n_huge;
  peer_wait(a.ps);
  for (int vr = warp0; vr < n_huge; vr += nwarps) {
    const int row = __ldg(a.row_order + vr);
    const int first = __ldg(a.hub_first + vr);
    const int deg = __ldg(a.rowptr + row + 1) - __ldg(a.rowptr + row);
    const int nch = a.seg ? __ldg(a.seg_cnt + vr) : (deg + SRB_HUB_CHUNK - 1) / SRB_HUB_CHUNK;
    float4 acc0 = f4_zero(), acc1 = f4_zero();
    for (int c = grp; c < nch; c += RPW) {
      const float* src = a.hub_part + (size_t)(first + c) * D + gl * 4;
      acc0 = f4_add(acc0, *reinterpret_cast<const float4*>(src));
      acc1 = f4_add(acc1, *reinterpret_cast<const float4*>(src + D / 2));
    }
    xor_reduce_groups(acc0, acc1, LPR);
    spmm_epilogue<D>(a, row, gl, acc0, acc1, grp == 0);
  }
}

template <int D, bool MASKED>
__global__ void __launch_bounds__(256) spmm_csr_kernel(const SpmmArgs a) {
  constexpr int LPR = D / 8;
  constexpr int RPW = 32 / LPR;
  const int lane = threadIdx.x & 31;
  const int wib = threadIdx.x >> 5;
  const int grp = lane / LPR;
  const int gl = lane % LPR;
  const int warp0 = (blockIdx.x * blockDim.x + threadIdx.x) >> 5;
  const int nwarps = (gridDim.x * blockDim.x) >> 5;

  pdl_wait();
  pdl_trigger();
  peer_wait(a.ps);
  int n_vlong = a.n_vlong, n_long = a.n_long, n_short = a.n_rows - a.n_huge - a.n_vlong - a.n_long;
  const int32_t* ro_v = a.row_order ? a.row_order + a.n_huge : nullptr;
  const int32_t* ro_l = a.row_order ? ro_v + n_vlong : nullptr;
  const int32_t* ro_s = a.row_order ? ro_l + n_long : nullptr;
  int id_l = n_vlong, id_s = n_vlong + n_long;
  if (a.n_vlong_dev) {
    n_vlong = min(a.n_vlong_dev[1], a.n_rows);
    n_long = min(a.n_vlong_dev[2], a.n_rows);
    n_short = min(a.n_vlong_dev[3], a.n_rows);
    ro_v = a.row_order + a.n_rows;
    ro_l = a.row_order + 2 * a.n_rows;
    ro_s = a.row_order + 3 * a.n_rows;
  }
  __shared__ float4 part[8][2][LPR];
  for (int vr = blockIdx.x; vr < n_vlong; vr += gridDim.x) {
    const int row = ro_v ? __ldg(ro_v + vr) : vr;
    const int beg = __ldg(a.rowptr + row);
    const int end = __ldg(a.rowptr + row + 1);
    const int per = ((end - beg + 255) / 256) * 32;
    const int wbeg = beg + wib * per;
    const int wend = min(end, wbeg + per);
    float4 acc0 = f4_zero(), acc1 = f4_zero();
    spmm_gather<D, MASKED>(a, wbeg + grp * LPR, wend, 32, gl, acc0, acc1);
    xor_reduce_groups(acc0, acc1, LPR);
    if (grp == 0) {
      part[wib][0][gl] = acc0;
      part[wib][1][gl] = acc1;
    }
    __syncthreads();
    if (wib == 0) {
      acc0 = f4_zero();
      acc1 = f4_zero();
#pragma unroll
      for (int w = 0; w < 8; ++w) {
        acc0 = f4_add(acc0, part[w][0][gl]);
        acc1 = f4_add(acc1, part[w][1][gl]);
      }
      spmm_epilogue<D>(a, row, gl, acc0, acc1, grp == 0);
    }
    __syncthreads();
  }

  const int n_items = n_long + (n_short + RPW - 1) / RPW;
  for (int item = warp0; item < n_items; item += nwarps) {
    const bool is_long = item < n_long;
    const int k = is_long ? item : (item - n_long) * RPW + grp;
    bool valid = is_long || k < n_short;
    int row = 0, p = 0, end = 0;
    if (valid) {
      if (is_long) row = ro_l ? __ldg(ro_l + k) : id_l + k;
      else row = ro_s ? __ldg(ro_s + k) : id_s + k;
      p = __ldg(a.rowptr + row);
      end = __ldg(a.rowptr + row + 1);
    }
    if (is_long) p += grp * LPR;
    float4 acc0 = f4_zero(), acc1 = f4_zero();
    spmm_gather<D, MASKED>(a, p, end, is_long ? 32 : LPR, gl, acc0, acc1);
    if (is_long) {
      xor_reduce_groups(acc0, acc1, LPR);
      valid = valid && grp == 0;
    }
    spmm_epilogue<D>(a, row, gl, acc0, acc1, valid);
  }
  peer_signal(a.ps);
}

__device__ __forceinline__ float4 multimem_ld_reduce_add4(const float* mc) {
  float4 v;
  asm volatile("multimem.ld_reduce.relaxed.sys.global.add.v4.f32 {%0, %1, %2, %3}, [%4];"
               : "=f"(v.x), "=f"(v.y), "=f"(v.z), "=f"(v.w)
               : "l"(mc)
               : "memory");
  return v;
}

template <int D>
__global__ void __launch_bounds__(256) reduce_rows_kernel(const SpmmArgs a, const ReduceArgs r) {
  constexpr int LPR = D / 8;
  constexpr int RPW = 32 / LPR;
  constexpr int HALF = D / 2;
  const int lane = threadIdx.x & 31;
  const int grp = lane / LPR;
  const int gl = lane % LPR;
  const int warp0 = (blockIdx.x * blockDim.x + threadIdx.x) >> 5;
  const int nwarps = (gridDim.x * blockDim.x) >> 5;
  const int n_items = (r.n_slice + RPW - 1) / RPW;
  peer_wait(a.ps);
  if (r.mc_part) {
    constexpr int UN = 4;
    for (int item = warp0 * UN; item < n_items; item += nwarps * UN) {
      float4 p0[UN], p1[UN];
      bool ok[UN];
#pragma unroll
      for (int u = 0; u < UN; ++u) {
        const int k = (item + u) * RPW + grp;
        ok[u] = (item + u) < n_items && k < r.n_slice;
        if (ok[u] && r.mask) {
          const int row = r.slice_begin + k;
          ok[u] = (__ldg(r.mask + (row >> 5)) >> (row & 31)) & 1u;
        }
        p0[u] = p1[u] = f4_zero();
        if (ok[u]) {
          const float* src = r.mc_part + (size_t)(r.slice_begin + k) * D + gl * 4;
          p0[u] = multimem_ld_reduce_add4(src);
          p1[u] = multimem_ld_reduce_add4(src + HALF);
        }
      }
#pragma unroll
      for (int u = 0; u < UN; ++u) {
        if (!__any_sync(SRB_FULL_MASK, ok[u])) continue;
        spmm_epilogue<D>(a, r.slice_begin + (item + u) * RPW + grp, gl, p0[u], p1[u], ok[u]);
      }
    }
    peer_signal(a.ps);
    return;
  }
  for (int item = warp0; item < n_items; item += nwarps) {
    const int k = item * RPW + grp;
    bool valid = k < r.n_slice;
    if (r.mask) {
      const int row = r.slice_begin + k;
      valid = valid && ((__ldg(r.mask + (row >> 5)) >> (row & 31)) & 1u);
      if (!__any_sync(SRB_FULL_MASK, valid)) continue;
    }
    float4 acc0 = f4_zero(), acc1 = f4_zero();
    if (valid) {
      const float* src = r.stage + (size_t)k * D + gl * 4;
      const size_t plane = (size_t)r.stage_cap * D;
#pragma unroll 1
      for (int q = 0; q < r.world; q += 2) {
        const bool two = q + 1 < r.world;
        const float4 p0 = ldg4(src + (size_t)q * plane), p1 = ldg4(src + (size_t)q * plane + HALF);
        float4 p2 = f4_zero(), p3 = f4_zero();
        if (two) {
          p2 = ldg4(src + (size_t)(q + 1) * plane);
          p3 = ldg4(src + (size_t)(q + 1) * plane + HALF);
        }
        acc0 = f4_add(acc0, p0);
        acc1 = f4_add(acc1, p1);
        if (two) {
          acc0 = f4_add(acc0, p2);
          acc1 = f4_add(acc1, p3);
        }
      }
    }
    spmm_epilogue<D>(a, r.slice_begin + k, gl, acc0, acc1, valid);
  }
  peer_signal(a.ps);
}

template <int D>
__global__ void __launch_bounds__(256) rows_epilogue_kernel(const SpmmArgs a) {
  constexpr int LPR = D / 8;
  constexpr int RPW = 32 / LPR;
  constexpr int HALF = D / 2;
  const int lane = threadIdx.x & 31;
  const int grp = lane / LPR;
  const int gl = lane % LPR;
  const int warp0 = (blockIdx.x * blockDim.x + threadIdx.x) >> 5;
  const int nwarps = (gridDim.x * blockDim.x) >> 5;
  const int n_items = (a.n_rows + RPW - 1) / RPW;
  pdl_wait();
  pdl_trigger();
  for (int item = warp0; item < n_items; item += nwarps) {
    const int row = item * RPW + grp;
    const bool valid = row < a.n_rows;
    float4 acc0 = f4_zero(), acc1 = f4_zero();
    if (valid) {
      const float* src = a.X + (size_t)row * D + gl * 4;
      acc0 = a.stream ? __ldcs(reinterpret_cast<const float4*>(src)) : ldg4(src);
      acc1 = a.stream ? __ldcs(reinterpret_cast<const float4*>(src + HALF)) : ldg4(src + HALF);
    }
    spmm_epilogue<D>(a, row, gl, acc0, acc1, valid);
  }
}

int launch_rows_epilogue(const SpmmArgs& a, int d, cudaStream_t st) {
  if (a.n_rows <= 0) return SRB_OK;
  const int rpw = 32 / (d / 8);
  long long blocks = ((long long)(a.n_rows + rpw - 1) / rpw + 7) / 8;
  const long long cap = (long long)sm_count() * 8;
  if (blocks > cap) blocks = cap;
  if (blocks < 1) blocks = 1;
  switch (d) {
    case 32: return launch_kernel(rows_epilogue_kernel<32>, (int)blocks, 256, 0, st, "rows_epilogue_kernel", a);
    case 64: return launch_kernel(rows_epilogue_kernel<64>, (int)blocks, 256, 0, st, "rows_epilogue_kernel", a);
    case 128: return launch_kernel(rows_epilogue_kernel<128>, (int)blocks, 256, 0, st, "rows_epilogue_kernel", a);
    default: set_error("rows_epilogue: unsupported d=%d (32, 64, 128)", d); return SRB_ERR_ARG;
  }
}

int launch_reduce_rows(const SpmmArgs& a, const ReduceArgs& r, int d, cudaStream_t st) {
  if (r.n_slice <= 0) return SRB_OK;
  const int rpw = 32 / (d / 8);
  long long blocks = ((long long)(r.n_slice + rpw - 1) / rpw + 7) / 8;
  const long long cap = (long long)sm_count() * (r.small_grid ? 1 : 8);
  if (blocks > cap) blocks = cap;
  if (blocks < 1) blocks = 1;
  switch (d) {
    case 32: reduce_rows_kernel<32><<<(int)blocks, 256, 0, st>>>(a, r); break;
    case 64: reduce_rows_kernel<64><<<(int)blocks, 256, 0, st>>>(a, r); break;
    case 128: reduce_rows_kernel<128><<<(int)blocks, 256, 0, st>>>(a, r); break;
    default: set_error("reduce_rows: unsupported d=%d (32, 64, 128)", d); return SRB_ERR_ARG;
  }
  return post_launch("reduce_rows_kernel");
}

template <int D, bool M>
static int launch_spmm_dma(const SpmmArgs& a, int hub_blocks, int blocks, cudaStream_t st) {
  if (hub_blocks > 0) {
    if (a.seg && a.n_warp > 0) {
      const int wb = max(1, min((a.n_warp + 7) / 8, blocks));
      SRB_TRY(launch_kernel(spmm_seg_warp_kernel<D, M>, wb, 256, 0, st, "spmm_seg_warp_kernel", a));
    }
    SRB_TRY(launch_kernel(spmm_hub_kernel<D, M>, hub_blocks, 256, 0, st, "spmm_hub_kernel", a));
    const int nh = a.n_vlong_dev ? a.n_rows : a.n_huge;
    SRB_TRY(launch_kernel(spmm_hub_finish_kernel<D>, max(1, min((nh + 7) / 8, hub_blocks)), 256, 0, st, "spmm_hub_finish_kernel", a));
  }
  return launch_kernel(spmm_csr_kernel<D, M>, blocks, 256, 0, st, "spmm_csr_kernel", a);
}

template <int D>
static int launch_spmm_d(const SpmmArgs& a, int hub_blocks, int blocks, cudaStream_t st) {
  if (a.col_mask != nullptr) return launch_spmm_dma<D, true>(a, hub_blocks, blocks, st);
  return launch_spmm_dma<D, false>(a, hub_blocks, blocks, st);
}

int launch_spmm(const SpmmArgs& a, int d, cudaStream_t st) {
  if (a.n_rows == 0) return SRB_OK;
  const int threads = 256;
  const int rpw = 32 / (d / 8);
  const long long items = (long long)a.n_long + ((long long)a.n_rows - a.n_huge - a.n_vlong - a.n_long + rpw - 1) / rpw;
  long long blocks = (items + threads / 32 - 1) / (threads / 32);
  if (a.n_vlong_dev) blocks = ((long long)a.n_rows + threads / 32 - 1) / (threads / 32);
  if (blocks < a.n_vlong) blocks = a.n_vlong;
  const long long cap = (long long)sm_count() * 8;
  if (blocks > cap) blocks = cap;
  if (blocks < 1) blocks = 1;
  long long hub_blocks = a.seg ? (a.n_cta > 0 ? a.n_cta : (a.n_work > 0 ? 1 : 0)) : a.n_work;
  if (hub_blocks > cap) hub_blocks = cap;
  switch (d) {
    case 32: return launch_spmm_d<32>(a, (int)hub_blocks, (int)blocks, st);
    case 64: return launch_spmm_d<64>(a, (int)hub_blocks, (int)blocks, st);
    case 128: return launch_spmm_d<128>(a, (int)hub_blocks, (int)blocks, st);
    default: set_error("spmm: unsupported d=%d (32, 64, 128)", d); return SRB_ERR_ARG;
  }
}

int fill_args(const srb_spmm_desc* d, SpmmArgs& a) {
  SRB_REQUIRE(d != nullptr, "spmm: null desc");
  SRB_REQUIRE(d->rowptr && d->colidx && d->vals && d->X, "spmm: null CSR/X pointer");
  SRB_REQUIRE(d->n_rows >= 0 && d->n_cols >= 0, "spmm: negative shape");
  SRB_REQUIRE(d->noise_mode >= 0 && d->noise_mode <= 2, "spmm: bad noise_mode");
  SRB_REQUIRE(d->noise_mode != 1 || d->noise, "spmm: noise_mode 1 needs a noise tensor");
  SRB_REQUIRE(!d->adam_p || (d->adam_m && d->adam_v && d->adam_scalars), "spmm: incomplete adam pointers");
  SRB_REQUIRE(d->X != d->Y, "spmm: Y must not alias X");
  a.rowptr = d->rowptr;
  a.colidx = d->colidx;
  a.vals = d->vals;
  a.row_order = d->row_order;
  a.n_rows = d->n_rows;
  a.n_vlong_dev = d->row_order ? d->n_vlong_dev : nullptr;
  const bool hub = d->row_order && d->hub.n_work > 0 && (a.n_vlong_dev || d->hub.n_rows > 0);
  SRB_REQUIRE(!hub || (d->hub.first && (d->hub.work || d->hub.seg) && d->hub.part), "spmm: split-row lists incomplete");
  SRB_REQUIRE(!hub || d->hub.n_rows <= d->n_rows, "spmm: more split rows than rows");
  a.n_huge = (hub && !a.n_vlong_dev) ? d->hub.n_rows : 0;
  a.hub_first = hub ? d->hub.first : nullptr;
  a.hub_work = hub ? d->hub.work : nullptr;
  a.hub_part = hub ? d->hub.part : nullptr;
  a.n_work = hub ? d->hub.n_work : 0;
  const bool segs = hub && !a.n_vlong_dev && d->hub.seg != nullptr;
  SRB_REQUIRE(!segs || (d->hub.seg_cnt && (d->hub.n_cta == 0 || d->hub.order_cta) && (d->hub.n_warp == 0 || d->hub.order_warp)),
              "spmm: column-blocked split-row lists incomplete");
  a.seg = segs ? d->hub.seg : nullptr;
  a.seg_cnt = segs ? d->hub.seg_cnt : nullptr;
  a.order_cta = segs ? d->hub.order_cta : nullptr;
  a.order_warp = segs ? d->hub.order_warp : nullptr;
  a.n_cta = segs ? d->hub.n_cta : 0;
  a.n_warp = segs ? d->hub.n_warp : 0;
  const int rest = d->n_rows - a.n_huge;
  a.n_vlong = (d->row_order && d->n_vlong_rows > 0) ? (d->n_vlong_rows < rest ? d->n_vlong_rows : rest) : 0;
  a.col_mask = d->col_mask;
  a.n_long = (d->row_order && d->n_long_rows > 0) ? (d->n_long_rows < rest - a.n_vlong ? d->n_long_rows : rest - a.n_vlong) : 0;
  a.X = d->X;
  a.Y = d->Y;
  a.extra = d->extra;
  a.extra_scale = d->extra_scale;
  a.seed_mask = nullptr;
  a.seed = nullptr;
  a.noise_mode = d->noise_mode;
  a.noise = d->noise;
  a.eps = d->eps;
  a.pkey = make_uint2((uint32_t)d->philox_seed, (uint32_t)(d->philox_seed >> 32));
  a.poff = make_uint2((uint32_t)d->philox_offset, (uint32_t)(d->philox_offset >> 32));
  a.pstep = d->philox_step_dev;
  a.sum_in = d->sum_in;
  a.sum_add[0] = a.sum_add[1] = a.sum_add[2] = nullptr;
  a.sum_out = d->sum_out;
  a.sum_scale = d->sum_scale;
  a.ap = d->adam_p;
  a.am = d->adam_m;
  a.av = d->adam_v;
  a.ascal = d->adam_scalars;
  a.b2 = (float)d->beta2;
  a.w1 = (float)(1.0 - d->beta1);
  a.w2 = (float)(1.0 - d->beta2);
  a.aeps = d->adam_eps;
  a.world = 0;
  a.noise_row_base = 0;
  a.noise_row_stride = 1;
  a.peer_mc = 0;
  a.ps = PeerSync{};
  a.stream = ((long long)d->n_rows + d->n_cols) * d->d * 4 > l2_bytes() / 4 * 3;
  a.stage_rank = a.stage_cap = 0;
  for (int g = 0; g < 8; ++g) a.peer[g] = a.peer_sum[g] = a.peer_p[g] = a.stage_peer[g] = nullptr;
  for (int g = 0; g < 9; ++g) a.stage_bounds[g] = 0;
  return SRB_OK;
}

int graph_args(const srb_graph_csr& g, int n_rows, int n_cols, int d, const float* X, SpmmArgs& a) {
  srb_spmm_desc p = {};
  p.rowptr = g.rowptr;
  p.colidx = g.colidx;
  p.vals = g.vals;
  p.row_order = g.row_order;
  p.n_long_rows = g.n_long_rows;
  p.n_vlong_rows = g.n_vlong_rows;
  p.hub = g.hub;
  p.n_rows = n_rows;
  p.n_cols = n_cols;
  p.d = d;
  p.X = X;
  p.extra_scale = 1.f;
  p.sum_scale = 1.f;
  return fill_args(&p, a);
}

}

extern "C" int srb_spmm_csr(const srb_spmm_desc* desc, void* stream) {
  srb::SpmmArgs a;
  SRB_TRY(srb::fill_args(desc, a));
  return srb::launch_spmm(a, desc->d, (cudaStream_t)stream);
}

extern "C" int srb_spmm_epilogue_rows(const srb_spmm_desc* desc, void* stream) {
  srb::SpmmArgs a;
  SRB_TRY(srb::fill_args(desc, a));
  SRB_REQUIRE(desc->Y || desc->sum_out || desc->adam_p, "spmm_epilogue_rows: nothing to write");
  return srb::launch_rows_epilogue(a, desc->d, (cudaStream_t)stream);
}

extern "C" int srb_encoder_forward(const srb_encoder_desc* e, void* stream) {
  SRB_REQUIRE(e != nullptr, "encoder: null desc");
  SRB_REQUIRE(e->E0 && e->final_out, "encoder: null E0/final_out");
  SRB_REQUIRE(e->n_layers >= 0, "encoder: negative n_layers");
  SRB_REQUIRE(e->n_layers == 0 || (e->work0 && e->work1), "encoder: work buffers required");
  SRB_REQUIRE(e->include_ego || e->n_layers > 0, "encoder: mean over zero layers");
  SRB_REQUIRE(!e->last_rows || (e->last_rows_out && e->last_rows_out != e->final_out && e->last_rows_out != e->E0),
              "encoder: last_rows needs a separate last_rows_out buffer");
  const size_t nd = (size_t)e->n * e->d;
  cudaStream_t st = (cudaStream_t)stream;
  const int L = e->n_layers;
  if (L == 0) {
    SRB_TRY(srb::check_cuda(cudaMemcpyAsync(e->final_out, e->E0, nd * 4, cudaMemcpyDeviceToDevice, st), "encoder copy"));
    if (e->cl_out)
      SRB_TRY(srb::check_cuda(cudaMemcpyAsync(e->cl_out, e->E0, nd * 4, cudaMemcpyDeviceToDevice, st), "encoder copy"));
    return SRB_OK;
  }
  const float inv = 1.0f / (float)(e->include_ego ? L + 1 : L);
  const bool want_cl = e->cl_out != nullptr;
  const bool cl_hit = want_cl && e->layer_cl >= 1 && e->layer_cl <= L;
  if (want_cl && !cl_hit)
    SRB_TRY(srb::check_cuda(cudaMemcpyAsync(e->cl_out, e->E0, nd * 4, cudaMemcpyDeviceToDevice, st), "encoder copy"));
  const float* x = e->E0;
  int k0 = 0;
  if (e->x1) {
    SRB_REQUIRE(L >= 2 && !e->include_ego && !(cl_hit && e->layer_cl == 1) && e->x1 != e->work0 && e->x1 != e->work1,
                "encoder: x1 needs n_layers >= 2, include_ego == 0, layer_cl != 1 and a buffer of its own");
    x = e->x1;
    k0 = 1;
  }
  const bool last_on_rows = e->last_rows && e->n_last_rows > 0 && !(cl_hit && e->layer_cl == L);
  const float* src[4];
  int n_src = 0;
  bool live = true;
  if (e->include_ego) src[n_src++] = e->E0;
  const float* px = e->E0;
  for (int k = 0; k < L - 1 && live; ++k) {
    const float* py = (k == 0 && e->x1) ? e->x1 : (cl_hit && k == e->layer_cl - 1) ? e->cl_out : (px == e->work0 ? e->work1 : e->work0);
    for (int j = 0; j < n_src; ++j) live = live && src[j] != py;
    live = live && n_src < 4;
    if (live) src[n_src++] = py;
    px = py;
  }
  const bool batch_mean = last_on_rows && live;
  for (int k = k0; k < L; ++k) {
    srb_spmm_desc s = {};
    s.rowptr = e->rowptr;
    s.colidx = e->colidx;
    s.vals = e->vals;
    s.row_order = e->row_order;
    s.n_long_rows = e->n_long_rows;
    s.n_vlong_rows = e->n_vlong_rows;
    s.hub = e->hub;
    s.n_rows = e->n;
    s.n_cols = e->n;
    s.d = e->d;
    s.X = x;
    const bool last = (k == L - 1);
    float* y = nullptr;
    if (cl_hit && k == e->layer_cl - 1) y = e->cl_out;
    else if (!last) y = (x == e->work0) ? e->work1 : e->work0;
    s.Y = y;
    s.noise_mode = e->noise_mode;
    if (e->noise_mode == 1) s.noise = e->noise + (size_t)k * nd;
    s.eps = e->eps;
    s.philox_seed = e->philox_seed;
    s.philox_offset = e->philox_offset + (uint64_t)k;
    s.philox_step_dev = e->philox_step_dev;
    s.sum_in = (k == 0) ? (e->include_ego ? e->E0 : nullptr) : ((k == 1 && e->x1) ? e->x1 : e->final_out);
    s.sum_out = (batch_mean && !last) ? nullptr : e->final_out;
    s.sum_scale = last ? inv : 1.0f;
    if (batch_mean && last) s.sum_in = n_src ? src[0] : nullptr;
    if (last && last_on_rows) {
      s.row_order = e->last_rows;
      s.n_rows = e->n_last_rows;
      if (e->last_rows_nv_dev) {
        s.n_vlong_rows = 0;
        s.n_long_rows = 0;
        s.n_vlong_dev = e->last_rows_nv_dev;
        s.hub = e->last_rows_hub;
      } else {
        s.n_vlong_rows = e->n_last_rows;
        s.n_long_rows = 0;
        s.hub = srb_hub_split{};
      }
      s.Y = nullptr;
      s.sum_out = e->last_rows_out;
    }
    srb::SpmmArgs a;
    SRB_TRY(srb::fill_args(&s, a));
    if (batch_mean && last)
      for (int j = 1; j < n_src; ++j) a.sum_add[j - 1] = src[j];
    SRB_TRY(srb::launch_spmm(a, s.d, st));
    x = y;
  }
  return SRB_OK;
}
```

selfrec_b200/csrc/spmm_args.cuh:

```cuda
#pragma once
#include "common.cuh"

namespace srb {

struct PeerSync {
  int* flags[8];
  int* epoch;
  int* counter;
  int* err;
  int world, rank;
  int wait, signal;
};

__device__ __forceinline__ void st_release_sys(int* p, int v) { asm volatile("st.release.sys.global.s32 [%0], %1;" ::"l"(p), "r"(v) : "memory"); }
__device__ __forceinline__ int ld_acquire_sys(const int* p) {
  int v;
  asm volatile("ld.acquire.sys.global.s32 %0, [%1];" : "=r"(v) : "l"(p) : "memory");
  return v;
}

__device__ __forceinline__ int ld_relaxed_sys(const int* p) {
  int v;
  asm volatile("ld.relaxed.sys.global.s32 %0, [%1];" : "=r"(v) : "l"(p) : "memory");
  return v;
}

__device__ __forceinline__ void peer_wait(const PeerSync& s) {
  if (!s.wait) return;
  if ((int)threadIdx.x < s.world) {
    const int target = *reinterpret_cast<volatile int*>(s.epoch);
    const int* f = s.flags[s.rank] + threadIdx.x;
    const long long t0 = clock64();
    while (ld_relaxed_sys(f) < target) {
      if (clock64() - t0 > 60000000000ll) {
        *s.err = 1;
        break;
      }
      __nanosleep(20);
    }
    (void)ld_acquire_sys(f);
  }
  __syncthreads();
}

__device__ __forceinline__ void peer_signal(const PeerSync& s) {
  if (!s.signal) return;
  __syncthreads();
  if (threadIdx.x == 0) {
    __threadfence();
    if (atomicAdd(s.counter, 1) == (int)gridDim.x - 1) {
      *s.counter = 0;
      __threadfence_system();
      const int e = *s.epoch + 1;
      *s.epoch = e;
      for (int q = 0; q < s.world; ++q) st_release_sys(s.flags[q] + s.rank, e);
    }
  }
}

struct SpmmArgs {
  const int32_t* rowptr;
  const int32_t* colidx;
  const float* vals;
  const int32_t* row_order;
  int32_t n_rows;
  const int32_t* n_vlong_dev;
  const uint32_t* col_mask;
  int32_t n_huge;
  int32_t n_vlong;
  int32_t n_long;
  const int32_t* hub_first;
  const int32_t* hub_work;
  int32_t n_work;
  float* hub_part;
  const int32_t* seg;
  const int32_t* seg_cnt;
  const int32_t* order_cta;
  const int32_t* order_warp;
  int32_t n_cta;
  int32_t n_warp;
  const float* X;
  float* Y;
  const float* extra;
  float extra_scale;
  const uint32_t* seed_mask;
  const float* seed;
  int32_t noise_mode;
  const float* noise;
  float eps;
  uint2 pkey;
  uint2 poff;
  const int32_t* pstep;
  const float* sum_in;
  const float* sum_add[3];
  float* sum_out;
  float sum_scale;
  float* ap;
  float* am;
  float* av;
  const float* ascal;
  float b2, w1, w2, aeps;
  int32_t world;
  float* peer[8];
  float* peer_sum[8];
  float* peer_p[8];
  int32_t stream;
  int32_t peer_mc;
  int32_t noise_row_base;
  int32_t noise_row_stride;
  float* stage_peer[8];
  int32_t stage_bounds[9];
  int32_t stage_rank;
  int32_t stage_cap;
  PeerSync ps;
};

struct ReduceArgs {
  const float* stage;
  int32_t world;
  int32_t stage_cap;
  int32_t slice_begin;
  int32_t n_slice;
  const uint32_t* mask;
  const float* mc_part;
  int32_t small_grid;
};

int launch_spmm(const SpmmArgs& a, int d, cudaStream_t st);
int launch_reduce_rows(const SpmmArgs& a, const ReduceArgs& r, int d, cudaStream_t st);
int launch_rows_epilogue(const SpmmArgs& a, int d, cudaStream_t st);
int fill_args(const srb_spmm_desc* d, SpmmArgs& a);
int graph_args(const srb_graph_csr& g, int n_rows, int n_cols, int d, const float* X, SpmmArgs& a);

inline uint64_t noise_offset(int view, int layer) { return ((uint64_t)view << 32) | (uint64_t)(0x10 + layer); }

__device__ __forceinline__ void list_batch_row(int row, int deg, int key_off, int32_t* rows, int cap, int32_t* counters,
                                               int32_t* hub_first, int32_t* hub_work, int hub_cap) {
  const int cls = (hub_first && deg >= SRB_HUB_MIN_NNZ) ? 0 : (deg >= 128 ? 1 : 2);
  const unsigned mine = __match_any_sync(__activemask(), cls + key_off);
  const int lane = threadIdx.x & 31;
  const int leader = __ffs(mine) - 1;
  int base = 0;
  if (lane == leader) base = atomicAdd(counters + cls, __popc(mine));
  base = __shfl_sync(mine, base, leader);
  const int slot = base + __popc(mine & ((1u << lane) - 1));
  rows[cls * cap + slot] = row;
  if (cls == 0) {
    const int nch = (deg + SRB_HUB_CHUNK - 1) / SRB_HUB_CHUNK;
    const int first = atomicAdd(counters + 4, nch);
    hub_first[slot] = first;
    for (int c = 0; c < nch && first + c < hub_cap; ++c) {
      hub_work[2 * (first + c)] = row;
      hub_work[2 * (first + c) + 1] = c;
    }
  }
}



}
```

Before: 1899.

## Overlap batch-row build, NCE view-2 prep and BPR scatter on side stream

Moves build_batch_rows onto a forked side stream that joins before encoder layer 1. For XSimGCL it also launches the InfoNCE prep for the contrastive view on the side stream once layer_cl is reached, so it runs alongside the remaining encoder layers. The BPR loss, its seed scatter and the finalize kernel run on the side stream concurrently with the InfoNCE main pass. This adds event record/wait overhead and more stream coordination in exchange for overlapping small kernels that were previously serialized.

Result: faster. 1920 (median of 6 runs) (+1.1%).

```diff
diff --git a/selfrec_b200/csrc/common.cuh b/selfrec_b200/csrc/common.cuh
--- a/selfrec_b200/csrc/common.cuh
+++ b/selfrec_b200/csrc/common.cuh
@@ -96,7 +96,8 @@
   const float *nce_u[2], *nce_i[2];
   const int32_t *cat, *n_cat;
 };
-int seed_segments(int model, int n_layers, int layer_cl, const SeedGrads& g, const SeedRows& r, ScatterSegs& segs);
+enum { SEED_ALL = 0, SEED_BPR = 1, SEED_NCE = 2 };
+int seed_segments(int model, int n_layers, int layer_cl, const SeedGrads& g, const SeedRows& r, ScatterSegs& segs, int part = SEED_ALL);
 int step_begin(int32_t* step, float* scalars, double lr, double b1, double b2, int32_t* words, int n_words, const int32_t* batch, int cap,
                int d, float* seed, int n_seed, const SeedRows& r, cudaStream_t st);
 
@@ -118,10 +119,16 @@
   int64_t nce_ws_bytes;
   float* losses;
 };
+enum { NCE_ALL = 0, NCE_PREP_VIEW2 = 1, NCE_AFTER_VIEW2 = 2 };
+int infonce_run(const srb_infonce_desc* d, int phase, cudaStream_t st);
+
+void nce_problems(int model, float tau, float cl_rate, int d, int cap, const float* out, const float* v1, const float* v2,
+                  const LossRows& r, const LossBufs& o, srb_infonce_desc& q, SeedGrads& g);
 struct ForkRes;
 int step_losses(int model, float reg, float l2_div, float tau, float cl_rate, int d, int cap, const float* out, const float* e0,
                 const float* v1, const float* v2, const LossRows& r, const LossBufs& o, ForkRes* fork,
-                const std::function<int()>& before_nce, SeedGrads& g, cudaStream_t st);
+                const std::function<int()>& before_nce, SeedGrads& g, cudaStream_t st, int nce_phase = NCE_ALL,
+                const std::function<int()>& after_bpr = nullptr);
 
 __device__ __forceinline__ void adam_prepare(int32_t* step, float* scalars, double lr, double b1, double b2) {
   const int t = *step + 1;
diff --git a/selfrec_b200/csrc/engine.cu b/selfrec_b200/csrc/engine.cu
--- a/selfrec_b200/csrc/engine.cu
+++ b/selfrec_b200/csrc/engine.cu
@@ -194,20 +194,25 @@
   out[3] = bpr_losses[0] + bpr_losses[1] + cl;
 }
 
-int seed_segments(int model, int n_layers, int layer_cl, const SeedGrads& g, const SeedRows& r, ScatterSegs& segs) {
+int seed_segments(int model, int n_layers, int layer_cl, const SeedGrads& g, const SeedRows& r, ScatterSegs& segs, int part) {
   const int B = g.cap, L = n_layers;
   const size_t plane = (size_t)B * g.d;
   const int32_t* rows = g.batch + SRB_BATCH_HEADER;
   const int32_t* n_dev = g.batch;
   const float cm = 1.f / (float)((model == SRB_MODEL_LIGHTGCN || model == SRB_MODEL_SGL) ? L + 1 : L);
   segs.count = 0;
+  bool in_bpr = false;
   auto add = [&](int t, bool item, const float* src, const int32_t* idx, const int32_t* n, int cap, float scale) {
+    if (part != SEED_ALL && in_bpr != (part == SEED_BPR)) return false;
     segs.s[segs.count++] = {src, idx, n, cap, item ? r.item_off[t] : r.user_off[t], scale, item ? 0 : r.user_mod, item ? 0 : r.user_rem};
+    return true;
   };
   auto add_bpr = [&](int t, const float* src, float scale) {
+    in_bpr = true;
     add(t, false, src, rows, n_dev, B, scale);
     add(t, true, src + plane, rows + B, n_dev, B, scale);
     add(t, true, src + 2 * plane, rows + 2 * B, n_dev, B, scale);
+    in_bpr = false;
   };
   auto add_nce = [&](int t, int view, float scale) {
     add(t, false, g.nce_u[view], rows + 3 * B, n_dev + 1, B, scale);
@@ -236,7 +241,7 @@
       break;
     case SRB_MODEL_SGL:
       for (int t = 0; t < 2; ++t) {
-        add(t, false, g.nce_u[t], g.cat, g.n_cat, 2 * B, cm);
+        if (!add(t, false, g.nce_u[t], g.cat, g.n_cat, 2 * B, cm)) continue;
         segs.s[segs.count - 1].item_min = r.item_min;
         segs.s[segs.count - 1].item_off = r.item_min > 0 ? r.item_off[t] : 0;
       }
@@ -274,6 +279,15 @@
   cudaEvent_t fork, join;
   bool ok;
 };
+static int fork_side(ForkRes* f, cudaStream_t st) {
+  SRB_TRY(check_cuda(cudaEventRecord(f->fork, st), "fork record"));
+  return check_cuda(cudaStreamWaitEvent(f->side, f->fork, 0), "fork wait");
+}
+static int join_side(ForkRes* f, cudaStream_t st) {
+  SRB_TRY(check_cuda(cudaEventRecord(f->join, f->side), "join record"));
+  return check_cuda(cudaStreamWaitEvent(st, f->join, 0), "join wait");
+}
+
 static ForkRes* fork_res(const srb_step_desc* s, ForkRes* own) {
   if (s->fork_stream && s->fork_event && s->join_event) {
     own->side = (cudaStream_t)s->fork_stream;
@@ -297,39 +311,11 @@
   return &r;
 }
 
-int step_losses(int model, float reg, float l2_div, float tau, float cl_rate, int d, int cap, const float* out, const float* e0,
-                const float* v1, const float* v2, const LossRows& r, const LossBufs& o, ForkRes* fork,
-                const std::function<int()>& before_nce, SeedGrads& g, cudaStream_t st) {
-  const bool lg = model == SRB_MODEL_LIGHTGCN, xs = model == SRB_MODEL_XSIMGCL, sg = model == SRB_MODEL_SIMGCL;
-  if (fork) {
-    SRB_TRY(check_cuda(cudaEventRecord(fork->fork, st), "fork record"));
-    SRB_TRY(check_cuda(cudaStreamWaitEvent(fork->side, fork->fork, 0), "fork wait"));
-  }
-  srb_bpr_desc p = {};
-  p.emb = out;
-  p.l2_emb = lg ? e0 : out;
-  p.n_users = r.item_off;
-  p.d = d;
-  p.u_idx = r.u;
-  p.i_idx = r.i;
-  p.j_idx = r.j;
-  p.b_dev = r.batch;
-  p.b = cap;
-  p.emb_scale = 1.f;
-  p.reg = reg;
-  p.l2_terms = (sg || xs) ? 2 : 3;
-  p.l2_div = l2_div;
-  p.grad_scale = 1.f;
-  p.losses = o.bpr_losses;
-  p.g_emb = o.g_emb;
-  p.g_l2 = lg ? o.g_l2 : nullptr;
-  p.scratch = o.bpr_scratch;
-  SRB_TRY(srb_bpr_l2_fwd_bwd(&p, fork ? fork->side : st));
-  if (fork) SRB_TRY(check_cuda(cudaEventRecord(fork->join, fork->side), "join record"));
-  if (before_nce) SRB_TRY(before_nce());
-
-  g = SeedGrads{r.batch, cap, d, o.g_emb, p.g_l2, {}, {}, nullptr, nullptr};
-  srb_infonce_desc q = {};
+void nce_problems(int model, float tau, float cl_rate, int d, int cap, const float* out, const float* v1, const float* v2,
+                  const LossRows& r, const LossBufs& o, srb_infonce_desc& q, SeedGrads& g) {
+  const bool xs = model == SRB_MODEL_XSIMGCL, sg = model == SRB_MODEL_SIMGCL;
+  g = SeedGrads{r.batch, cap, d, o.g_emb, model == SRB_MODEL_LIGHTGCN ? o.g_l2 : nullptr, {}, {}, nullptr, nullptr};
+  q = {};
   q.d = d;
   q.b_cos = 1;
   q.temperature = tau;
@@ -356,10 +342,48 @@
     g.cat = r.cat_id;
     g.n_cat = r.n_cat;
   }
-  if (q.n_problems) SRB_TRY(srb_infonce_fwd_bwd(&q, st));
-  if (fork) SRB_TRY(check_cuda(cudaStreamWaitEvent(st, fork->join, 0), "join wait"));
-  return launch_kernel(finalize_losses_kernel, 1, 1, 0, st, "finalize_losses_kernel", o.bpr_losses, o.nce_losses, q.n_problems, cl_rate,
-                       o.losses);
+}
+
+int step_losses(int model, float reg, float l2_div, float tau, float cl_rate, int d, int cap, const float* out, const float* e0,
+                const float* v1, const float* v2, const LossRows& r, const LossBufs& o, ForkRes* fork,
+                const std::function<int()>& before_nce, SeedGrads& g, cudaStream_t st, int nce_phase,
+                const std::function<int()>& after_bpr) {
+  const bool lg = model == SRB_MODEL_LIGHTGCN, xs = model == SRB_MODEL_XSIMGCL, sg = model == SRB_MODEL_SIMGCL;
+  srb_infonce_desc q;
+  nce_problems(model, tau, cl_rate, d, cap, out, v1, v2, r, o, q, g);
+  if (fork) {
+    if (nce_phase == NCE_AFTER_VIEW2) SRB_TRY(join_side(fork, st));
+    SRB_TRY(fork_side(fork, st));
+  }
+  srb_bpr_desc p = {};
+  p.emb = out;
+  p.l2_emb = lg ? e0 : out;
+  p.n_users = r.item_off;
+  p.d = d;
+  p.u_idx = r.u;
+  p.i_idx = r.i;
+  p.j_idx = r.j;
+  p.b_dev = r.batch;
+  p.b = cap;
+  p.emb_scale = 1.f;
+  p.reg = reg;
+  p.l2_terms = (sg || xs) ? 2 : 3;
+  p.l2_div = l2_div;
+  p.grad_scale = 1.f;
+  p.losses = o.bpr_losses;
+  p.g_emb = o.g_emb;
+  p.g_l2 = lg ? o.g_l2 : nullptr;
+  p.scratch = o.bpr_scratch;
+  SRB_TRY(srb_bpr_l2_fwd_bwd(&p, fork ? fork->side : st));
+  if (after_bpr) SRB_TRY(after_bpr());
+  if (before_nce) SRB_TRY(before_nce());
+  if (q.n_problems) SRB_TRY(infonce_run(&q, nce_phase, st));
+  if (fork) {
+    SRB_TRY(join_side(fork, st));
+    SRB_TRY(fork_side(fork, st));
+  }
+  return launch_kernel(finalize_losses_kernel, 1, 1, 0, fork ? fork->side : st, "finalize_losses_kernel", o.bpr_losses, o.nce_losses,
+                       q.n_problems, cl_rate, o.losses);
 }
 
 static int run_chain(const srb_step_desc* s, const Ws& w, const srb_graph_csr* g, const float* F, const float* G, int g_level,
@@ -381,7 +405,8 @@
 }
 
 static int encoder(const srb_step_desc* s, const Ws& w, const srb_graph_csr* g, bool include_ego, int noise_mode, int view,
-                   int layer_cl, float* final_out, float* cl_out, cudaStream_t st, const float* x1 = nullptr) {
+                   int layer_cl, float* final_out, float* cl_out, cudaStream_t st, const float* x1 = nullptr,
+                   const std::function<int(int)>& before_layer = nullptr) {
   srb_encoder_desc e = {};
   e.rowptr = g->rowptr;
   e.colidx = g->colidx;
@@ -416,7 +441,7 @@
   e.work0 = w.work0;
   e.work1 = w.work1;
   e.x1 = x1;
-  return srb_encoder_forward(&e, st);
+  return encoder_forward(&e, st, before_layer);
 }
 
 static int perturb_rows(const srb_step_desc* s, const float* x, float* out, int view, cudaStream_t st) {
@@ -474,12 +499,36 @@
   const SeedRows rows = {{0, N, 2 * N}, {U, N + U, 2 * N + U}, 0, 0};
 
   PdlScope pdl;
-
+  ForkRes fk_own = {};
+  ForkRes* fk = s->model != SRB_MODEL_MF ? fork_res(s, &fk_own) : nullptr;
+  const bool has_nce = s->model == SRB_MODEL_XSIMGCL || s->model == SRB_MODEL_SIMGCL || s->model == SRB_MODEL_SGL;
+  const LossRows lr = {s->batch, u_idx, i_idx, j_idx, U, uq_u, uq_i, {0, U}, w.idx_cat, w.n_cat, w.idx_cat};
+  const LossBufs lb = {w.g_emb, w.g_l2, w.g_nce, (size_t)2 * B * d, w.bpr_scratch, w.bpr_losses, w.nce_losses, w.nce_ws, w.nce_ws_bytes, s->losses};
+
+  const bool rows_aside = fk && L >= 2;
+  const bool cl_aside = fk && s->model == SRB_MODEL_XSIMGCL && s->layer_cl >= 1 && s->layer_cl < L;
+  bool rows_pending = rows_aside;
+  std::function<int(int)> before_layer;
   if (s->model != SRB_MODEL_MF) {
     const int n_words = 8 + (U + s->n_items + 31) / 32;
     SRB_TRY(step_begin(s->step_dev, s->scalars, s->lr, s->beta1, s->beta2, w.n_hub, n_words, s->batch, B, d, w.seed, w.n_seed, rows, st));
-    SRB_TRY(launch_kernel(build_batch_rows_kernel, (3 * B + 255) / 256, 256, 0, st, "build_batch_rows_kernel", s->batch, B, U, s->adj.rowptr,
-                          w.batch_rows, w.n_hub, w.row_mask, w.hub_cap ? w.hub_first : nullptr, w.hub_work, w.hub_cap));
+    if (rows_aside) SRB_TRY(fork_side(fk, st));
+    SRB_TRY(launch_kernel(build_batch_rows_kernel, (3 * B + 255) / 256, 256, 0, rows_aside ? fk->side : st, "build_batch_rows_kernel", s->batch,
+                          B, U, s->adj.rowptr, w.batch_rows, w.n_hub, w.row_mask, w.hub_cap ? w.hub_first : nullptr, w.hub_work, w.hub_cap));
+    before_layer = [&](int k) {
+      if (k == 1 && rows_pending) {
+        SRB_TRY(join_side(fk, st));
+        rows_pending = false;
+      }
+      if (k == s->layer_cl && cl_aside) {
+        srb_infonce_desc q;
+        SeedGrads g;
+        nce_problems(s->model, s->tau, s->cl_rate, d, B, w.final_, w.cl, w.v2, lr, lb, q, g);
+        SRB_TRY(fork_side(fk, st));
+        SRB_TRY(infonce_run(&q, NCE_PREP_VIEW2, fk->side));
+      }
+      return (int)SRB_OK;
+    };
   } else {
     SRB_TRY(srb_adam_prepare(s->step_dev, s->scalars, s->lr, s->beta1, s->beta2, stream));
   }
@@ -487,13 +536,13 @@
   switch (s->model) {
     case SRB_MODEL_MF: break;
     case SRB_MODEL_LIGHTGCN:
-      SRB_TRY(encoder(s, w, &s->adj, true, 0, 0, 0, w.final_, nullptr, st));
+      SRB_TRY(encoder(s, w, &s->adj, true, 0, 0, 0, w.final_, nullptr, st, nullptr, before_layer));
       table = w.final_;
       break;
     case SRB_MODEL_XSIMGCL:
       SRB_REQUIRE(s->noise_mode == 1 || s->noise_mode == 2, "step: XSimGCL needs noise_mode 1 or 2");
       SRB_REQUIRE(s->noise_mode != 1 || s->noise, "step: noise tensor missing");
-      SRB_TRY(encoder(s, w, &s->adj, false, s->noise_mode, 0, s->layer_cl, w.final_, w.cl, st));
+      SRB_TRY(encoder(s, w, &s->adj, false, s->noise_mode, 0, s->layer_cl, w.final_, w.cl, st, nullptr, before_layer));
       table = w.final_;
       break;
     case SRB_MODEL_SIMGCL:
@@ -503,11 +552,11 @@
         SRB_TRY(spmm_simple(s, &s->adj, s->params, w.acc0, nullptr, false, st));
         SRB_TRY(perturb_rows(s, w.acc0, w.acc1, 0, st));
         SRB_TRY(perturb_rows(s, w.acc0, w.gd, 1, st));
-        SRB_TRY(encoder(s, w, &s->adj, false, 0, 0, 0, w.final_, nullptr, st, w.acc0));
-        SRB_TRY(encoder(s, w, &s->adj, false, s->noise_mode, 0, 0, w.cl, nullptr, st, w.acc1));
-        SRB_TRY(encoder(s, w, &s->adj, false, s->noise_mode, 1, 0, w.v2, nullptr, st, w.gd));
+        SRB_TRY(encoder(s, w, &s->adj, false, 0, 0, 0, w.final_, nullptr, st, w.acc0, before_layer));
+        SRB_TRY(encoder(s, w, &s->adj, false, s->noise_mode, 0, 0, w.cl, nullptr, st, w.acc1, before_layer));
+        SRB_TRY(encoder(s, w, &s->adj, false, s->noise_mode, 1, 0, w.v2, nullptr, st, w.gd, before_layer));
       } else {
-        SRB_TRY(encoder(s, w, &s->adj, false, 0, 0, 0, w.final_, nullptr, st));
+        SRB_TRY(encoder(s, w, &s->adj, false, 0, 0, 0, w.final_, nullptr, st, nullptr, before_layer));
         SRB_TRY(encoder(s, w, &s->adj, false, s->noise_mode, 0, 0, w.cl, nullptr, st));
         SRB_TRY(encoder(s, w, &s->adj, false, s->noise_mode, 1, 0, w.v2, nullptr, st));
       }
@@ -515,22 +564,27 @@
       break;
     case SRB_MODEL_SGL:
       SRB_REQUIRE(s->adj_view[0].rowptr && s->adj_view[1].rowptr, "step: SGL needs two view graphs");
-      SRB_TRY(encoder(s, w, &s->adj, true, 0, 0, 0, w.final_, nullptr, st));
+      SRB_TRY(encoder(s, w, &s->adj, true, 0, 0, 0, w.final_, nullptr, st, nullptr, before_layer));
       SRB_TRY(encoder(s, w, &s->adj_view[0], true, 0, 0, 0, w.cl, nullptr, st));
-      SRB_TRY(encoder(s, w, &s->adj_view[1], true, 0, 0, 0, w.v2, nullptr, st));
+      SRB_TRY(encoder(s, w, &s->adj_view[1], true, 0, 0, 0, w.v2, nullptr, st, nullptr, before_layer));
       table = w.final_;
       break;
   }
 
-  ForkRes fk_own = {};
-  ForkRes* fk = (s->model == SRB_MODEL_XSIMGCL || s->model == SRB_MODEL_SIMGCL || s->model == SRB_MODEL_SGL) ? fork_res(s, &fk_own) : nullptr;
+  ForkRes* fkl = has_nce ? fk : nullptr;
   std::function<int()> build_cat;
   if (s->model == SRB_MODEL_SGL)
     build_cat = [&] { return launch_kernel(build_cat_idx_kernel, 8, 256, 0, st, "build_cat_idx_kernel", s->batch, B, U, w.idx_cat, w.n_cat); };
-  const LossRows lr = {s->batch, u_idx, i_idx, j_idx, U, uq_u, uq_i, {0, U}, w.idx_cat, w.n_cat, w.idx_cat};
-  const LossBufs lb = {w.g_emb, w.g_l2, w.g_nce, (size_t)2 * B * d, w.bpr_scratch, w.bpr_losses, w.nce_losses, w.nce_ws, w.nce_ws_bytes, s->losses};
   SeedGrads gr;
-  SRB_TRY(step_losses(s->model, s->reg, s->l2_div, s->tau, s->cl_rate, d, B, table, s->params, w.cl, w.v2, lr, lb, fk, build_cat, gr, st));
+  std::function<int()> scatter_bpr;
+  if (fkl)
+    scatter_bpr = [&] {
+      ScatterSegs sg = {};
+      seed_segments(s->model, L, s->layer_cl, gr, rows, sg, SEED_BPR);
+      return scatter_segments(w.seed, d, sg, fkl->side);
+    };
+  SRB_TRY(step_losses(s->model, s->reg, s->l2_div, s->tau, s->cl_rate, d, B, table, s->params, w.cl, w.v2, lr, lb, fkl, build_cat, gr, st,
+                      cl_aside ? NCE_AFTER_VIEW2 : NCE_ALL, scatter_bpr));
 
   const size_t plane = (size_t)B * d;
   if (s->model == SRB_MODEL_MF) {
@@ -547,12 +601,15 @@
   }
   auto seed_table = [&](int t) { return w.seed + (size_t)t * N * d; };
   ScatterSegs sg = {};
-  const int g_level = seed_segments(s->model, L, s->layer_cl, gr, rows, sg);
+  const int g_level = seed_segments(s->model, L, s->layer_cl, gr, rows, sg, fkl ? SEED_NCE : SEED_ALL);
   SRB_TRY(scatter_segments(w.seed, d, sg, st));
-  if (s->model != SRB_MODEL_SGL)
-    return run_chain(s, w, &s->adj, seed_table(0), g_level >= 0 ? seed_table(1) : nullptr, g_level, s->model == SRB_MODEL_LIGHTGCN,
-                     nullptr, nullptr, st);
-  SRB_TRY(run_chain(s, w, &s->adj_view[0], seed_table(0), nullptr, -1, true, w.gd, nullptr, st));
-  SRB_TRY(run_chain(s, w, &s->adj_view[1], seed_table(1), nullptr, -1, true, w.gd, w.gd, st));
-  return run_chain(s, w, &s->adj, seed_table(2), nullptr, -1, true, nullptr, w.gd, st);
-}
+  if (s->model != SRB_MODEL_SGL) {
+    SRB_TRY(run_chain(s, w, &s->adj, seed_table(0), g_level >= 0 ? seed_table(1) : nullptr, g_level, s->model == SRB_MODEL_LIGHTGCN,
+                      nullptr, nullptr, st));
+  } else {
+    SRB_TRY(run_chain(s, w, &s->adj_view[0], seed_table(0), nullptr, -1, true, w.gd, nullptr, st));
+    SRB_TRY(run_chain(s, w, &s->adj_view[1], seed_table(1), nullptr, -1, true, w.gd, w.gd, st));
+    SRB_TRY(run_chain(s, w, &s->adj, seed_table(2), nullptr, -1, true, nullptr, w.gd, st));
+  }
+  return fkl ? join_side(fkl, st) : SRB_OK;
+}
diff --git a/selfrec_b200/csrc/infonce.cu b/selfrec_b200/csrc/infonce.cu
--- a/selfrec_b200/csrc/infonce.cu
+++ b/selfrec_b200/csrc/infonce.cu
@@ -5,6 +5,7 @@
 
 constexpr int NCE_T = 64;
 constexpr int NCE_MAX_SPLITS = 8;
+constexpr int NCE_VIEW1 = 1, NCE_VIEW2 = 2;
 
 struct NceProblem {
   const float* table1;
@@ -51,15 +52,16 @@
 __device__ __forceinline__ int nce_n(const NceProblem& p) { return p.n_dev ? min(*p.n_dev, p.n) : p.n; }
 
 template <int D>
-__global__ void __launch_bounds__(256) nce_prep_kernel(const NceArgs a) {
+__global__ void __launch_bounds__(256) nce_prep_kernel(const NceArgs a, const int views) {
   pdl_wait();
   pdl_trigger();
   const NceProblem& p = a.p[blockIdx.y];
+  const bool do1 = views & NCE_VIEW1, do2 = views & NCE_VIEW2;
   const int lane = threadIdx.x & 31;
   const int i = blockIdx.x * (blockDim.x >> 5) + (threadIdx.x >> 5);
   if (i >= a.np) return;
   const int n = nce_n(p);
-  if (blockIdx.x == 0 && threadIdx.x == 0) *p.loss_acc = 0.f;
+  if (do1 && blockIdx.x == 0 && threadIdx.x == 0) *p.loss_acc = 0.f;
   constexpr int Q = (D + 127) / 128;
   float4 v1[Q], v2[Q];
   float s1 = 0.f, s2 = 0.f, s12 = 0.f;
@@ -68,8 +70,8 @@
 #pragma unroll
     for (int q = 0; q < Q; ++q) {
       const int c = lane * 4 + q * 128;
-      v1[q] = (c < D) ? f4_scale(p.scale1, ldg4(p.table1 + (size_t)(r + p.row_off1) * D + c)) : f4_zero();
-      v2[q] = (c < D) ? f4_scale(p.scale2, ldg4(p.table2 + (size_t)(r + p.row_off2) * D + c)) : f4_zero();
+      v1[q] = (c < D && do1) ? f4_scale(p.scale1, ldg4(p.table1 + (size_t)(r + p.row_off1) * D + c)) : f4_zero();
+      v2[q] = (c < D && do2) ? f4_scale(p.scale2, ldg4(p.table2 + (size_t)(r + p.row_off2) * D + c)) : f4_zero();
       s1 += f4_dot(v1[q], v1[q]);
       s2 += f4_dot(v2[q], v2[q]);
     }
@@ -92,16 +94,19 @@
       v1[q] = make_float4(v1[q].x / n1, v1[q].y / n1, v1[q].z / n1, v1[q].w / n1);
       v2[q] = make_float4(v2[q].x / n2, v2[q].y / n2, v2[q].z / n2, v2[q].w / n2);
     }
+    if (!do2 && c < D) v2[q] = *reinterpret_cast<const float4*>(p.V2 + (size_t)i * D + c);
     s12 += f4_dot(v1[q], v2[q]);
-    if (c < D) {
+    if (c < D && do1) {
       st4(p.V1 + (size_t)i * D + c, v1[q]);
-      st4(p.V2 + (size_t)i * D + c, v2[q]);
       st4(p.dV1 + (size_t)i * D + c, f4_zero());
-      st4(p.dV2 + (size_t)i * D + c, f4_zero());
       p.V1T[(size_t)(c + 0) * a.np + i] = v1[q].x;
       p.V1T[(size_t)(c + 1) * a.np + i] = v1[q].y;
       p.V1T[(size_t)(c + 2) * a.np + i] = v1[q].z;
       p.V1T[(size_t)(c + 3) * a.np + i] = v1[q].w;
+    }
+    if (c < D && do2) {
+      st4(p.V2 + (size_t)i * D + c, v2[q]);
+      st4(p.dV2 + (size_t)i * D + c, f4_zero());
       p.V2T[(size_t)(c + 0) * a.np + i] = v2[q].x;
       p.V2T[(size_t)(c + 1) * a.np + i] = v2[q].y;
       p.V2T[(size_t)(c + 2) * a.np + i] = v2[q].z;
@@ -110,36 +115,47 @@
   }
   s12 = warp_sum(s12);
   if (lane == 0) {
-    p.inv1[i] = i1;
-    p.inv2[i] = i2;
-    p.diag[i] = s12 * a.inv_tau;
-  }
-}
-
-__global__ void __launch_bounds__(256) nce_prep_tc_kernel(const NceArgs a) {
+    if (do2) p.inv2[i] = i2;
+    if (do1) {
+      p.inv1[i] = i1;
+      p.diag[i] = s12 * a.inv_tau;
+    }
+  }
+}
+
+__global__ void __launch_bounds__(256) nce_prep_tc_kernel(const NceArgs a, const int views) {
   pdl_wait();
   pdl_trigger();
   constexpr int D = 64;
   __shared__ float t1[32][D + 1], t2[32][D + 1];
   const NceProblem& p = a.p[blockIdx.y];
+  const bool do1 = views & NCE_VIEW1, do2 = views & NCE_VIEW2;
   const int lane = threadIdx.x & 31, warp = threadIdx.x >> 5;
   const int i0 = blockIdx.x * 32;
   const int n = nce_n(p);
-  if (blockIdx.x == 0 && threadIdx.x == 0) *p.loss_acc = 0.f;
+  if (do1 && blockIdx.x == 0 && threadIdx.x == 0) *p.loss_acc = 0.f;
   const size_t nd = (size_t)a.np * D;
   float* hi = p.dV2 + nd;
   float* lo = hi + 4 * nd;
-#pragma unroll 1
+  const int c = lane * 2;
+  float2 w1[4], w2[4];
+#pragma unroll
+  for (int rr = 0; rr < 4; ++rr) {
+    const int i = i0 + warp * 4 + rr;
+    w1[rr] = w2[rr] = make_float2(0.f, 0.f);
+    if (i < n) {
+      const int r = p.idx[i];
+      if (do1) w1[rr] = *reinterpret_cast<const float2*>(p.table1 + (size_t)(r + p.row_off1) * D + c);
+      if (do2) w2[rr] = *reinterpret_cast<const float2*>(p.table2 + (size_t)(r + p.row_off2) * D + c);
+    }
+    if (!do2) w2[rr] = *reinterpret_cast<const float2*>(p.V2 + (size_t)i * D + c);
+  }
+#pragma unroll
   for (int rr = 0; rr < 4; ++rr) {
     const int il = warp * 4 + rr, i = i0 + il;
-    const int c = lane * 2;
-    float2 v1 = make_float2(0.f, 0.f), v2 = make_float2(0.f, 0.f);
-    if (i < n) {
-      const int r = p.idx[i];
-      v1 = *reinterpret_cast<const float2*>(p.table1 + (size_t)(r + p.row_off1) * D + c);
-      v2 = *reinterpret_cast<const float2*>(p.table2 + (size_t)(r + p.row_off2) * D + c);
-      v1.x *= p.scale1, v1.y *= p.scale1, v2.x *= p.scale2, v2.y *= p.scale2;
-    }
+    float2 v1 = w1[rr], v2 = make_float2(0.f, 0.f);
+    v1.x *= p.scale1, v1.y *= p.scale1;
+    if (do2) v2 = make_float2(w2[rr].x * p.scale2, w2[rr].y * p.scale2);
     const float s1 = warp_sum(v1.x * v1.x + v1.y * v1.y);
     const float s2 = warp_sum(v2.x * v2.x + v2.y * v2.y);
     float i1 = 1.f, i2 = 1.f;
@@ -148,22 +164,28 @@
       i1 = 1.f / n1, i2 = 1.f / n2;
       v1.x /= n1, v1.y /= n1, v2.x /= n2, v2.y /= n2;
     }
+    const size_t o = (size_t)i * D + c;
+    if (!do2) v2 = w2[rr];
     const float s12 = warp_sum(v1.x * v2.x + v1.y * v2.y);
-    const size_t o = (size_t)i * D + c;
-    *reinterpret_cast<float2*>(p.V1 + o) = v1;
-    *reinterpret_cast<float2*>(p.V2 + o) = v2;
-    *reinterpret_cast<float2*>(p.dV1 + o) = make_float2(0.f, 0.f);
-    *reinterpret_cast<float2*>(p.dV2 + o) = make_float2(0.f, 0.f);
-    const float2 h1 = make_float2(tf32_rna(v1.x), tf32_rna(v1.y)), h2 = make_float2(tf32_rna(v2.x), tf32_rna(v2.y));
-    *reinterpret_cast<float2*>(hi + o) = h1;
-    *reinterpret_cast<float2*>(hi + nd + o) = h2;
-    *reinterpret_cast<float2*>(lo + o) = make_float2(v1.x - h1.x, v1.y - h1.y);
-    *reinterpret_cast<float2*>(lo + nd + o) = make_float2(v2.x - h2.x, v2.y - h2.y);
-    t1[il][c] = v1.x, t1[il][c + 1] = v1.y;
-    t2[il][c] = v2.x, t2[il][c + 1] = v2.y;
-    if (lane == 0) {
+    if (do1) {
+      const float2 h1 = make_float2(tf32_rna(v1.x), tf32_rna(v1.y));
+      *reinterpret_cast<float2*>(p.V1 + o) = v1;
+      *reinterpret_cast<float2*>(p.dV1 + o) = make_float2(0.f, 0.f);
+      *reinterpret_cast<float2*>(hi + o) = h1;
+      *reinterpret_cast<float2*>(lo + o) = make_float2(v1.x - h1.x, v1.y - h1.y);
+      t1[il][c] = v1.x, t1[il][c + 1] = v1.y;
+    }
+    if (do2) {
+      const float2 h2 = make_float2(tf32_rna(v2.x), tf32_rna(v2.y));
+      *reinterpret_cast<float2*>(p.V2 + o) = v2;
+      *reinterpret_cast<float2*>(p.dV2 + o) = make_float2(0.f, 0.f);
+      *reinterpret_cast<float2*>(hi + nd + o) = h2;
+      *reinterpret_cast<float2*>(lo + nd + o) = make_float2(v2.x - h2.x, v2.y - h2.y);
+      t2[il][c] = v2.x, t2[il][c + 1] = v2.y;
+    }
+    if (lane == 0 && do2) p.inv2[i] = i2;
+    if (lane == 0 && do1) {
       p.inv1[i] = i1;
-      p.inv2[i] = i2;
       const float dg = s12 * a.inv_tau;
       p.diag[i] = dg;
       p.part_l[i] = expf(dg - a.inv_tau);
@@ -173,12 +195,16 @@
   for (int e = threadIdx.x; e < D * 32; e += 256) {
     const int dc = e >> 5, il = e & 31;
     const size_t o = (size_t)dc * a.np + i0 + nce_tperm(il);
-    const float x1 = t1[il][dc], x2 = t2[il][dc];
-    const float g1 = tf32_rna(x1), g2 = tf32_rna(x2);
-    hi[2 * nd + o] = g1;
-    hi[3 * nd + o] = g2;
-    lo[2 * nd + o] = x1 - g1;
-    lo[3 * nd + o] = x2 - g2;
+    if (do1) {
+      const float x1 = t1[il][dc], g1 = tf32_rna(x1);
+      hi[2 * nd + o] = g1;
+      lo[2 * nd + o] = x1 - g1;
+    }
+    if (do2) {
+      const float x2 = t2[il][dc], g2 = tf32_rna(x2);
+      hi[3 * nd + o] = g2;
+      lo[3 * nd + o] = x2 - g2;
+    }
   }
 }
 
@@ -497,12 +523,15 @@
   }
 }
 
-static int nce_launch_tc(const NceArgs& a, int n_problems, cudaStream_t st) {
+static int prep_views(int phase) { return phase == NCE_PREP_VIEW2 ? NCE_VIEW2 : (phase == NCE_AFTER_VIEW2 ? NCE_VIEW1 : NCE_VIEW1 | NCE_VIEW2); }
+
+static int nce_launch_tc(const NceArgs& a, int n_problems, int phase, cudaStream_t st) {
   const int np = a.np;
   const int d = NT_D;
   {
     dim3 grid(np / 32, n_problems);
-    SRB_TRY(launch_kernel(nce_prep_tc_kernel, grid, 256, 0, st, "nce_prep_tc_kernel", a));
+    SRB_TRY(launch_kernel(nce_prep_tc_kernel, grid, 256, 0, st, "nce_prep_tc_kernel", a, prep_views(phase)));
+    if (phase == NCE_PREP_VIEW2) return SRB_OK;
   }
   NtMaps maps;
   NtArgs t;
@@ -564,11 +593,12 @@
 }
 
 template <int D>
-static int nce_launch(const NceArgs& a, int n_problems, cudaStream_t st) {
+static int nce_launch(const NceArgs& a, int n_problems, int phase, cudaStream_t st) {
   const int np = a.np;
   {
     dim3 grid((np + 7) / 8, n_problems);
-    SRB_TRY(launch_kernel(nce_prep_kernel<D>, grid, 256, 0, st, "nce_prep_kernel", a));
+    SRB_TRY(launch_kernel(nce_prep_kernel<D>, grid, 256, 0, st, "nce_prep_kernel", a, prep_views(phase)));
+    if (phase == NCE_PREP_VIEW2) return SRB_OK;
   }
   {
     static bool attr_done = false;
@@ -595,7 +625,9 @@
   return srb::nce_problem_floats(srb::nce_np(max_n), d) * 4 * n_problems;
 }
 
-extern "C" int srb_infonce_fwd_bwd(const srb_infonce_desc* d, void* stream) {
+namespace srb {
+
+int infonce_run(const srb_infonce_desc* d, int phase, cudaStream_t stream) {
   SRB_REQUIRE(d != nullptr, "infonce: null desc");
   SRB_REQUIRE(d->n_problems >= 1 && d->n_problems <= 4, "infonce: n_problems must be 1..4");
   SRB_REQUIRE(d->temperature > 0.f, "infonce: temperature must be positive");
@@ -611,26 +643,27 @@
               "infonce: workspace too small (%lld < %lld)", (long long)d->workspace_bytes,
               (long long)srb_infonce_workspace_bytes(max_n, d->d, d->n_problems));
   if (max_n == 0) {
+    if (phase == NCE_PREP_VIEW2) return SRB_OK;
     for (int q = 0; q < d->n_problems; ++q)
-      SRB_TRY(srb::check_cuda(cudaMemsetAsync(d->prob[q].loss, 0, 4, (cudaStream_t)stream), "infonce memset"));
+      SRB_TRY(check_cuda(cudaMemsetAsync(d->prob[q].loss, 0, 4, stream), "infonce memset"));
     return SRB_OK;
   }
-  srb::NceArgs a;
+  NceArgs a;
   a.n_problems = d->n_problems;
-  a.np = srb::nce_np(max_n);
+  a.np = nce_np(max_n);
   a.b_cos = d->b_cos;
   a.inv_tau = 1.0f / d->temperature;
-  const int row_blocks = a.np / srb::NCE_T;
-  int splits = (2 * srb::sm_count() + row_blocks * d->n_problems - 1) / (row_blocks * d->n_problems);
+  const int row_blocks = a.np / NCE_T;
+  int splits = (2 * sm_count() + row_blocks * d->n_problems - 1) / (row_blocks * d->n_problems);
   if (splits < 1) splits = 1;
-  if (splits > srb::NCE_MAX_SPLITS) splits = srb::NCE_MAX_SPLITS;
+  if (splits > NCE_MAX_SPLITS) splits = NCE_MAX_SPLITS;
   if (splits > row_blocks) splits = row_blocks;
   a.splits = splits;
   float* w = reinterpret_cast<float*>(d->workspace);
-  const int64_t per = srb::nce_problem_floats(a.np, d->d);
+  const int64_t per = nce_problem_floats(a.np, d->d);
   for (int q = 0; q < d->n_problems; ++q) {
     const srb_infonce_problem& s = d->prob[q];
-    srb::NceProblem& p = a.p[q];
+    NceProblem& p = a.p[q];
     p.table1 = s.table1;
     p.table2 = s.table2;
     p.row_off1 = s.row_off1;
@@ -657,15 +690,19 @@
     p.inv2 = t + a.np;
     p.diag = t + 2 * a.np;
     p.part_m = t + 3 * a.np;
-    p.part_l = t + 3 * a.np + (int64_t)srb::NCE_MAX_SPLITS * a.np;
-    p.lse = t + 3 * a.np + 2ll * srb::NCE_MAX_SPLITS * a.np;
+    p.part_l = t + 3 * a.np + (int64_t)NCE_MAX_SPLITS * a.np;
+    p.lse = t + 3 * a.np + 2ll * NCE_MAX_SPLITS * a.np;
     p.loss_acc = p.lse + a.np;
   }
-  cudaStream_t st = (cudaStream_t)stream;
-  if (d->d == 64 && d->b_cos && d->n_problems <= 2 && a.inv_tau <= 40.f) return srb::nce_launch_tc(a, d->n_problems, st);
+  cudaStream_t st = stream;
+  if (d->d == 64 && d->b_cos && d->n_problems <= 2 && a.inv_tau <= 40.f) return nce_launch_tc(a, d->n_problems, phase, st);
   switch (d->d) {
-    case 32: return srb::nce_launch<32>(a, d->n_problems, st);
-    case 64: return srb::nce_launch<64>(a, d->n_problems, st);
-    default: return srb::nce_launch<128>(a, d->n_problems, st);
-  }
-}
+    case 32: return nce_launch<32>(a, d->n_problems, phase, st);
+    case 64: return nce_launch<64>(a, d->n_problems, phase, st);
+    default: return nce_launch<128>(a, d->n_problems, phase, st);
+  }
+}
+
+}
+
+extern "C" int srb_infonce_fwd_bwd(const srb_infonce_desc* d, void* stream) { return srb::infonce_run(d, srb::NCE_ALL, (cudaStream_t)stream); }
diff --git a/selfrec_b200/csrc/spmm.cu b/selfrec_b200/csrc/spmm.cu
--- a/selfrec_b200/csrc/spmm.cu
+++ b/selfrec_b200/csrc/spmm.cu
@@ -698,7 +698,9 @@
   return srb::launch_rows_epilogue(a, desc->d, (cudaStream_t)stream);
 }
 
-extern "C" int srb_encoder_forward(const srb_encoder_desc* e, void* stream) {
+namespace srb {
+
+int encoder_forward(const srb_encoder_desc* e, cudaStream_t st, const std::function<int(int)>& before_layer) {
   SRB_REQUIRE(e != nullptr, "encoder: null desc");
   SRB_REQUIRE(e->E0 && e->final_out, "encoder: null E0/final_out");
   SRB_REQUIRE(e->n_layers >= 0, "encoder: negative n_layers");
@@ -707,7 +709,6 @@
   SRB_REQUIRE(!e->last_rows || (e->last_rows_out && e->last_rows_out != e->final_out && e->last_rows_out != e->E0),
               "encoder: last_rows needs a separate last_rows_out buffer");
   const size_t nd = (size_t)e->n * e->d;
-  cudaStream_t st = (cudaStream_t)stream;
   const int L = e->n_layers;
   if (L == 0) {
     SRB_TRY(srb::check_cuda(cudaMemcpyAsync(e->final_out, e->E0, nd * 4, cudaMemcpyDeviceToDevice, st), "encoder copy"));
@@ -743,6 +744,7 @@
   }
   const bool batch_mean = last_on_rows && live;
   for (int k = k0; k < L; ++k) {
+    if (before_layer) SRB_TRY(before_layer(k));
     srb_spmm_desc s = {};
     s.rowptr = e->rowptr;
     s.colidx = e->colidx;
@@ -795,3 +797,7 @@
   }
   return SRB_OK;
 }
+
+}
+
+extern "C" int srb_encoder_forward(const srb_encoder_desc* e, void* stream) { return srb::encoder_forward(e, (cudaStream_t)stream, nullptr); }
diff --git a/selfrec_b200/csrc/spmm_args.cuh b/selfrec_b200/csrc/spmm_args.cuh
--- a/selfrec_b200/csrc/spmm_args.cuh
+++ b/selfrec_b200/csrc/spmm_args.cuh
@@ -132,6 +132,8 @@
 int fill_args(const srb_spmm_desc* d, SpmmArgs& a);
 int graph_args(const srb_graph_csr& g, int n_rows, int n_cols, int d, const float* X, SpmmArgs& a);
 
+int encoder_forward(const srb_encoder_desc* e, cudaStream_t st, const std::function<int(int)>& before_layer);
+
 inline uint64_t noise_offset(int view, int layer) { return ((uint64_t)view << 32) | (uint64_t)(0x10 + layer); }
 
 __device__ __forceinline__ void list_batch_row(int row, int deg, int key_off, int32_t* rows, int cap, int32_t* counters,
```
